# tiberiu44/TTS-Cube

Hardware: NVIDIA B200
Metric: audio samples/sec (higher is better)
Workload: dtype f32 in/out; tcgen05: fp16 hi*hi + 2 x fp8 (e4m3/e5m2) correction passes (GEMM1), split-fp16 x3 (GEMM2), f32 accumulate

## Files before the change

### include/cube_vocoder.h

```cpp
#ifndef CUBE_VOCODER_H_
#define CUBE_VOCODER_H_

#include <stdint.h>

#ifdef __cplusplus
extern "C" {
#endif

typedef struct cube_voc cube_voc_t;
typedef void* cube_stream_t;

enum cube_voc_arch {
  CUBE_VOC_HIFIGAN = 0,
  CUBE_VOC_PWN_STUDENT = 1,
  CUBE_VOC_WAVERNN = 2,
  CUBE_VOC_UPSAMPLENET = 3
};

enum cube_wavernn_head { CUBE_HEAD_MOL = 0, CUBE_HEAD_GM = 1, CUBE_HEAD_MULAW = 2, CUBE_HEAD_RAW = 3 };

enum cube_voc_math {
  CUBE_MATH_FP32_SIMT = 0,
  CUBE_MATH_TC_SPLIT16 = 1
};

#define CUBE_MAX_UPS 8
#define CUBE_MAX_RBK 8
#define CUBE_MAX_DIL 8
#define CUBE_MAX_FLOWS 8

typedef struct cube_voc_config {
  uint32_t struct_size;
  int32_t arch;
  int32_t math;
  int32_t num_mels;
  int32_t upsample_initial_channel;
  int32_t n_ups;
  int32_t upsample_rates[CUBE_MAX_UPS];
  int32_t upsample_kernel_sizes[CUBE_MAX_UPS];
  int32_t resblock_type;
  int32_t n_resblock_kernels;
  int32_t resblock_kernel_sizes[CUBE_MAX_RBK];
  int32_t n_dilations[CUBE_MAX_RBK];
  int32_t resblock_dilations[CUBE_MAX_RBK][CUBE_MAX_DIL];
  int32_t n_flows;
  int32_t flow_blocks[CUBE_MAX_FLOWS];
  int32_t res_channels, gate_channels, skip_channels;
  int32_t kernel_size, front_kernel;
  int32_t dilation_base, dilation_cycle;
  int32_t n_upsample;
  int32_t upsample_scales[4];
  int32_t wrnn_layers, wrnn_size;
  int32_t wrnn_upsample, wrnn_upsample_low;
  int32_t wrnn_use_lowres;
  int32_t wrnn_head;
} cube_voc_config;

int cube_voc_create(cube_voc_t** out, const cube_voc_config* cfg, int device);

int cube_voc_load_weight(cube_voc_t* h, const char* name, const float* data, const int64_t* shape, int ndim);

int cube_voc_finalize(cube_voc_t* h);

int64_t cube_voc_out_len(const cube_voc_t* h, int64_t n_frames);

int cube_voc_forward(cube_voc_t* h, const float* mel, const int32_t* n_frames, const float* noise,
                     float* wav, int16_t* wav_i16, int B, int64_t Fmax, cube_stream_t stream);

int cube_voc_hifigan_support(const cube_voc_config* cfg, int64_t s0, int64_t s1, int64_t* f0, int64_t* f1);

int cube_voc_forward_range(cube_voc_t* h, const float* mel, const int32_t* n_frames, const int64_t* out_begin,
                           const int64_t* out_end, float* wav, int16_t* wav_i16, int B, int64_t Fmax, cube_stream_t stream);

int cube_voc_forward_host(cube_voc_t* h, const float* mel, const int32_t* n_frames, const float* noise,
                          float* wav, int16_t* wav_i16, int B, int64_t Fmax);

int64_t cube_wavernn_out_len(const cube_voc_t* h, int64_t n_frames, int64_t n_low);
int cube_wavernn_forward(cube_voc_t* h, const float* mel, const float* x_low, const float* draws, float* x,
                         int B, int64_t F, int64_t Tl, cube_stream_t stream);
int cube_wavernn_max_batch(const cube_voc_t* h);

int cube_voc_get_cond(cube_voc_t* h, float* c_up, int B, int64_t Tmax, cube_stream_t stream);

int64_t cube_voc_last_launches(const cube_voc_t* h);
int64_t cube_voc_workspace_bytes(const cube_voc_t* h);
int cube_voc_set_profile(cube_voc_t* h, int on);
int cube_voc_get_profile(cube_voc_t* h, char* names , float* ms, int cap);

void cube_voc_destroy(cube_voc_t* h);
const char* cube_voc_last_error(void);
const char* cube_voc_build_info(void);

int cube_mulaw_encode(const float* x, int64_t* q, int64_t n, cube_stream_t stream);
int cube_mulaw_decode(const int64_t* q, float* x, int64_t n, cube_stream_t stream);
int cube_raw_encode(const float* x, int64_t* q, int64_t n, cube_stream_t stream);
int cube_raw_decode(const int64_t* q, float* x, int64_t n, cube_stream_t stream);
int cube_mol_sample(const float* y, const float* u_mix, const float* u_x, float* x, int64_t n,
                    int nr_mix, float log_scale_min, float temperature, cube_stream_t stream);
int cube_gaussian_sample(const float* y, const float* eps, float* x, int64_t n, cube_stream_t stream);
int cube_categorical_sample(const float* logits, const float* u, int64_t* idx, int64_t n, int C,
                            cube_stream_t stream);
int cube_wav_to_int16(const float* wav, int16_t* out, int64_t n, cube_stream_t stream);

typedef struct cube_mel cube_mel_t;

typedef struct cube_mel_config {
  uint32_t struct_size;
  int32_t n_fft;
  int32_t win_size;
  int32_t hop_size;
  int32_t n_mels;
  int32_t pad_left;
  int32_t pad_right;
  int32_t log10_out;
  int32_t layout;
  int32_t pad_mode;
  float mag_eps;
  float floor_val;
  float pad_value;
  float preemph;
} cube_mel_config;

int cube_mel_create(cube_mel_t** out, const cube_mel_config* cfg, const float* window, const float* mel_basis, int device);
int64_t cube_mel_out_frames(const cube_mel_t* h, int64_t n_samples);
int cube_mel_forward(cube_mel_t* h, const float* wav, const int32_t* n_samples, float* mel, int B, int64_t Tmax,
                     int64_t Fmax, cube_stream_t stream);
void cube_mel_destroy(cube_mel_t* h);

#ifdef __cplusplus
}
#endif
#endif
```

### tts_cube_b200/_lib.py

```python
from __future__ import annotations

import ctypes as C
import os

_HERE = os.path.dirname(os.path.abspath(__file__))
LIB_PATH = os.path.join(_HERE, "libcube_vocoder.so")

MAX_UPS, MAX_RBK, MAX_DIL, MAX_FLOWS = 8, 8, 8, 8
ARCH_HIFIGAN, ARCH_PWN_STUDENT, ARCH_WAVERNN, ARCH_UPSAMPLENET = 0, 1, 2, 3
HEADS = {"mol": 0, "gm": 1, "mulaw": 2, "raw": 3}
MATH_FP32_SIMT, MATH_TC_SPLIT16 = 0, 1


class VocConfig(C.Structure):
    _fields_ = [
        ("struct_size", C.c_uint32),
        ("arch", C.c_int32), ("math", C.c_int32), ("num_mels", C.c_int32),
        ("upsample_initial_channel", C.c_int32), ("n_ups", C.c_int32),
        ("upsample_rates", C.c_int32 * MAX_UPS), ("upsample_kernel_sizes", C.c_int32 * MAX_UPS),
        ("resblock_type", C.c_int32), ("n_resblock_kernels", C.c_int32),
        ("resblock_kernel_sizes", C.c_int32 * MAX_RBK), ("n_dilations", C.c_int32 * MAX_RBK),
        ("resblock_dilations", (C.c_int32 * MAX_DIL) * MAX_RBK),
        ("n_flows", C.c_int32), ("flow_blocks", C.c_int32 * MAX_FLOWS),
        ("res_channels", C.c_int32), ("gate_channels", C.c_int32), ("skip_channels", C.c_int32),
        ("kernel_size", C.c_int32), ("front_kernel", C.c_int32),
        ("dilation_base", C.c_int32), ("dilation_cycle", C.c_int32),
        ("n_upsample", C.c_int32), ("upsample_scales", C.c_int32 * 4),
        ("wrnn_layers", C.c_int32), ("wrnn_size", C.c_int32), ("wrnn_upsample", C.c_int32),
        ("wrnn_upsample_low", C.c_int32), ("wrnn_use_lowres", C.c_int32), ("wrnn_head", C.c_int32),
    ]

    def __init__(self, *a, **k):
        super().__init__(*a, **k)
        self.struct_size = C.sizeof(VocConfig)


class MelConfig(C.Structure):
    _fields_ = [("struct_size", C.c_uint32),
                ("n_fft", C.c_int32), ("win_size", C.c_int32), ("hop_size", C.c_int32), ("n_mels", C.c_int32),
                ("pad_left", C.c_int32), ("pad_right", C.c_int32), ("log10_out", C.c_int32), ("layout", C.c_int32),
                ("pad_mode", C.c_int32),
                ("mag_eps", C.c_float), ("floor_val", C.c_float), ("pad_value", C.c_float), ("preemph", C.c_float)]

    def __init__(self, *a, **k):
        super().__init__(*a, **k)
        self.struct_size = C.sizeof(MelConfig)


class CubeVocError(RuntimeError):
    pass


_lib = None

_P = C.c_void_p
SYMBOLS = {
    "cube_voc_create": (C.c_int, [C.POINTER(_P), C.POINTER(VocConfig), C.c_int]),
    "cube_voc_load_weight": (C.c_int, [_P, C.c_char_p, _P, C.POINTER(C.c_int64), C.c_int]),
    "cube_voc_finalize": (C.c_int, [_P]),
    "cube_voc_out_len": (C.c_int64, [_P, C.c_int64]),
    "cube_voc_forward": (C.c_int, [_P, _P, _P, _P, _P, _P, C.c_int, C.c_int64, _P]),
    "cube_voc_forward_host": (C.c_int, [_P, _P, _P, _P, _P, _P, C.c_int, C.c_int64]),
    "cube_voc_hifigan_support": (C.c_int, [C.POINTER(VocConfig), C.c_int64, C.c_int64, C.POINTER(C.c_int64),
                                           C.POINTER(C.c_int64)]),
    "cube_voc_forward_range": (C.c_int, [_P, _P, _P, C.POINTER(C.c_int64), C.POINTER(C.c_int64), _P, _P, C.c_int,
                                         C.c_int64, _P]),
    "cube_voc_get_cond": (C.c_int, [_P, _P, C.c_int, C.c_int64, _P]),
    "cube_wavernn_out_len": (C.c_int64, [_P, C.c_int64, C.c_int64]),
    "cube_wavernn_forward": (C.c_int, [_P, _P, _P, _P, _P, C.c_int, C.c_int64, C.c_int64, _P]),
    "cube_wavernn_max_batch": (C.c_int, [_P]),
    "cube_voc_last_launches": (C.c_int64, [_P]),
    "cube_voc_workspace_bytes": (C.c_int64, [_P]),
    "cube_voc_set_profile": (C.c_int, [_P, C.c_int]),
    "cube_voc_get_profile": (C.c_int, [_P, _P, _P, C.c_int]),
    "cube_voc_destroy": (None, [_P]),
    "cube_voc_last_error": (C.c_char_p, []),
    "cube_voc_build_info": (C.c_char_p, []),
    "cube_mulaw_encode": (C.c_int, [_P, _P, C.c_int64, _P]),
    "cube_mulaw_decode": (C.c_int, [_P, _P, C.c_int64, _P]),
    "cube_raw_encode": (C.c_int, [_P, _P, C.c_int64, _P]),
    "cube_raw_decode": (C.c_int, [_P, _P, C.c_int64, _P]),
    "cube_mol_sample": (C.c_int, [_P, _P, _P, _P, C.c_int64, C.c_int, C.c_float, C.c_float, _P]),
    "cube_gaussian_sample": (C.c_int, [_P, _P, _P, C.c_int64, _P]),
    "cube_categorical_sample": (C.c_int, [_P, _P, _P, C.c_int64, C.c_int, _P]),
    "cube_wav_to_int16": (C.c_int, [_P, _P, C.c_int64, _P]),
    "cube_mel_create": (C.c_int, [C.POINTER(_P), C.POINTER(MelConfig), _P, _P, C.c_int]),
    "cube_mel_out_frames": (C.c_int64, [_P, C.c_int64]),
    "cube_mel_forward": (C.c_int, [_P, _P, C.POINTER(C.c_int32), _P, C.c_int, C.c_int64, C.c_int64, _P]),
    "cube_mel_destroy": (None, [_P]),
}


def lib() -> C.CDLL:
    global _lib
    if _lib is None:
        if not os.path.exists(LIB_PATH):
            raise CubeVocError(
                f"{LIB_PATH} not found - build it with `python -c 'import __graft_entry__ as g; g.build()'` "
                "(nvcc, sm_100a).  tts_cube_b200 has no CPU or PyTorch fallback.")
        l = C.CDLL(LIB_PATH)
        for name, (res, args) in SYMBOLS.items():
            fn = getattr(l, name)
            fn.restype = res
            fn.argtypes = args
        _lib = l
    return _lib


def check(rc: int) -> None:
    if rc != 0:
        raise CubeVocError(lib().cube_voc_last_error().decode("utf-8", "replace"))


def build_info() -> str:
    return lib().cube_voc_build_info().decode()
```

### tts_cube_b200/csrc/engine.cu

```cuda
#include <cuda_runtime.h>
#include <math.h>
#include <stdarg.h>
#include <stdio.h>
#include <string.h>

#include <map>
#include <string>
#include <vector>

#include "../../include/cube_vocoder.h"
#include "conv_simt.cuh"
#include "heads.cuh"
#include "tc_conv.cuh"
#include "tc_block.cuh"
#include "tc_rbstep.cuh"
#include "wavernn.cuh"
#include "melspec.cuh"

#define CUBE_VERSION "0.1.0"
#ifndef CUBE_FUSED_DEFAULT
#define CUBE_FUSED_DEFAULT true
#endif

namespace cube {

static thread_local char g_err[1024] = "";

static int fail(const char* fmt, ...) {
  va_list ap;
  va_start(ap, fmt);
  vsnprintf(g_err, sizeof(g_err), fmt, ap);
  va_end(ap);
  return 1;
}

#define CU_TRY(expr)                                                                       \
  do {                                                                                     \
    cudaError_t _e = (expr);                                                               \
    if (_e != cudaSuccess)                                                                 \
      return fail("%s failed: %s (%s:%d)", #expr, cudaGetErrorString(_e), __FILE__, __LINE__); \
  } while (0)

struct HostTensor {
  std::vector<int64_t> shape;
  std::vector<float> data;
  int64_t numel() const { int64_t n = 1; for (auto s : shape) n *= s; return n; }
};

struct DevBuf {
  float* p = nullptr;
  size_t bytes = 0;
};

struct PackedConv {
  float* W = nullptr;
  float* bias = nullptr;
  int M = 0, Mpad = 0, Ktot = 0, nphase = 1;
};

struct ProfRec { std::string name; cudaEvent_t a, b; };

struct TcPacked {
  __half* Wimg = nullptr;
  uint8_t* Wimg8 = nullptr;
  float* inv_scale = nullptr;
  float* bias = nullptr;
  int N = 0, n_tiles = 0, nchunks_total = 0, nseg = 0;
  int bn = 256, nphase = 1;
  long long w_phase_stride = 0;
  tc::TcSeg seg[2];
};

}

using namespace cube;

struct cube_voc {
  cube_voc_config cfg;
  int device = 0;
  bool finalized = false;
  std::map<std::string, HostTensor> host_w;
  std::vector<void*> dev_allocs;
  std::map<std::string, DevBuf> ws;
  int* d_lens = nullptr; size_t lens_cap = 0;
  std::vector<int> h_lens;
  void* hs_in = nullptr; size_t hs_in_cap = 0;
  float* d_mel = nullptr; size_t d_mel_cap = 0;
  float* d_noise = nullptr; size_t d_noise_cap = 0;
  float* d_wav = nullptr; size_t d_wav_cap = 0;
  int16_t* d_wav16 = nullptr; size_t d_wav16_cap = 0;
  cudaStream_t own_stream = nullptr;
  int64_t launches = 0;
  struct GraphEntry { cudaGraphExec_t exec = nullptr; uint64_t gen = 0; int64_t launches = 0; int seen = 0; };
  std::map<std::vector<int64_t>, GraphEntry> graphs;
  uint64_t alloc_gen = 0;
  int* h_lens_pin = nullptr; size_t h_lens_pin_cap = 0;
  bool lens_from_pinned = false;
  int sm_count = 148;
  bool profile = false;
  std::vector<ProfRec> prof;
  PackedConv conv_pre, conv_post_w;
  std::vector<PackedConv> ups;
  std::vector<std::vector<PackedConv>> rb_c1, rb_c2;
  TcPacked tc_conv_pre;
  std::vector<TcPacked> tc_ups;
  std::vector<std::vector<TcPacked>> tc_c1, tc_c2;
  struct Flow {
    PackedConv front, final1, final3;
    std::vector<PackedConv> gate, resskip;
    std::vector<TcPacked> tc_gate, tc_resskip;
    TcPacked tc_final1;
    TcPacked tc_front;
    bool has_tc_front = false;
    float* w3 = nullptr;
  };
  std::vector<Flow> flows;
  struct Up2 { float w[192]; float bias; int s; };
  std::vector<Up2> up2;
  struct Wrnn {
    PackedConv lowres[3], gx;
    float *w_last = nullptr, *whh1 = nullptr, *bhh1 = nullptr, *wih2 = nullptr, *bih2 = nullptr, *whh2 = nullptr, *bhh2 = nullptr;
    float *wpre = nullptr, *bpre = nullptr, *wout = nullptr, *bout = nullptr;
    int S = 0, ic = 0;
  } wr;
  struct UpNet { PackedConv conv[3]; std::vector<PackedConv> up; std::vector<int> J; } upnet;
  int last_B = 0; int64_t last_T = 0;
  std::vector<int> h_rng;
};

namespace cube {

static int dev_upload(cube_voc* h, const std::vector<float>& v, float** out) {
  float* d = nullptr;
  CU_TRY(cudaMalloc(&d, std::max<size_t>(v.size(), 1) * sizeof(float)));
  CU_TRY(cudaMemcpy(d, v.data(), v.size() * sizeof(float), cudaMemcpyHostToDevice));
  h->dev_allocs.push_back(d);
  *out = d;
  return 0;
}

static int ws_get(cube_voc* h, const char* name, size_t n_floats, float** out) {
  DevBuf& b = h->ws[name];
  const size_t need = n_floats * sizeof(float);
  if (b.bytes < need) {
    if (b.p) CU_TRY(cudaFree(b.p));
    b.p = nullptr; b.bytes = 0;
    ++h->alloc_gen;
    CU_TRY(cudaMalloc(&b.p, need));
    b.bytes = need;
  }
  *out = b.p;
  return 0;
}

static int get_weight(cube_voc* h, const std::string& base, HostTensor* out) {
  auto it = h->host_w.find(base + ".weight");
  if (it != h->host_w.end()) { *out = it->second; return 0; }
  auto ig = h->host_w.find(base + ".weight_g"), iv = h->host_w.find(base + ".weight_v");
  if (ig == h->host_w.end() || iv == h->host_w.end()) return fail("missing weight '%s.weight[_g/_v]'", base.c_str());
  const HostTensor& g = ig->second; const HostTensor& v = iv->second;
  const int64_t n0 = v.shape[0], inner = v.numel() / n0;
  if (g.numel() != n0) return fail("weight_g of '%s' has %lld elements, expected %lld", base.c_str(), (long long)g.numel(), (long long)n0);
  out->shape = v.shape;
  out->data.resize(v.data.size());
  for (int64_t i = 0; i < n0; ++i) {
    double ss = 0;
    for (int64_t j = 0; j < inner; ++j) { double x = v.data[i * inner + j]; ss += x * x; }
    const float scale = (float)((double)g.data[i] / sqrt(ss));
    for (int64_t j = 0; j < inner; ++j) out->data[i * inner + j] = v.data[i * inner + j] * scale;
  }
  return 0;
}

static int get_bias(cube_voc* h, const std::string& base, int64_t n, const HostTensor** out) {
  auto it = h->host_w.find(base + ".bias");
  if (it == h->host_w.end()) return fail("missing '%s.bias'", base.c_str());
  if (it->second.numel() != n) return fail("'%s.bias' has %lld elements, expected %lld", base.c_str(), (long long)it->second.numel(), (long long)n);
  *out = &it->second;
  return 0;
}

static int expect_shape(const std::string& name, const HostTensor& t, std::initializer_list<int64_t> s) {
  std::vector<int64_t> e(s);
  if (t.shape != e) {
    std::string got, exp;
    for (auto x : t.shape) got += std::to_string(x) + ",";
    for (auto x : e) exp += std::to_string(x) + ",";
    return fail("weight '%s' has shape [%s], expected [%s]", name.c_str(), got.c_str(), exp.c_str());
  }
  return 0;
}

static inline int round_up(int x, int m) { return (x + m - 1) / m * m; }

static int pack_conv1d(cube_voc* h, const std::string& base, int M, int C, int K, PackedConv* pc) {
  HostTensor w; const HostTensor* b;
  if (get_weight(h, base, &w)) return 1;
  if (expect_shape(base, w, {M, C, K})) return 1;
  if (get_bias(h, base, M, &b)) return 1;
  pc->M = M; pc->Mpad = round_up(M, 128); pc->Ktot = C * K; pc->nphase = 1;
  std::vector<float> P((size_t)pc->Ktot * pc->Mpad, 0.f), B(pc->Mpad, 0.f);
  for (int m = 0; m < M; ++m) {
    B[m] = b->data[m];
    for (int c = 0; c < C; ++c)
      for (int k = 0; k < K; ++k) P[(size_t)(c * K + k) * pc->Mpad + m] = w.data[((size_t)m * C + c) * K + k];
  }
  if (dev_upload(h, P, &pc->W)) return 1;
  return dev_upload(h, B, &pc->bias);
}

static int pack_convT(cube_voc* h, const std::string& base, int C, int M, int K, int u, PackedConv* pc, int* J_out) {
  HostTensor w; const HostTensor* b;
  if (get_weight(h, base, &w)) return 1;
  if (expect_shape(base, w, {C, M, K})) return 1;
  if (get_bias(h, base, M, &b)) return 1;
  const int J = (K + u - 1) / u;
  pc->M = M; pc->Mpad = round_up(M, 128); pc->Ktot = C * J; pc->nphase = u;
  std::vector<float> P((size_t)u * pc->Ktot * pc->Mpad, 0.f), B(pc->Mpad, 0.f);
  for (int m = 0; m < M; ++m) B[m] = b->data[m];
  for (int r = 0; r < u; ++r)
    for (int c = 0; c < C; ++c)
      for (int jj = 0; jj < J; ++jj) {
        const int k = r + (J - 1 - jj) * u;
        if (k >= K) continue;
        for (int m = 0; m < M; ++m)
          P[((size_t)r * pc->Ktot + (size_t)c * J + jj) * pc->Mpad + m] = w.data[((size_t)c * M + m) * K + k];
      }
  *J_out = J;
  if (dev_upload(h, P, &pc->W)) return 1;
  return dev_upload(h, B, &pc->bias);
}

static int pack_small(cube_voc* h, const std::string& base, int M, int C, int K, PackedConv* pc) {
  HostTensor w; const HostTensor* b;
  if (get_weight(h, base, &w)) return 1;
  if (expect_shape(base, w, {M, C, K})) return 1;
  if (get_bias(h, base, M, &b)) return 1;
  pc->M = M; pc->Mpad = M; pc->Ktot = C * K;
  std::vector<float> P((size_t)C * K * M), B(M);
  for (int m = 0; m < M; ++m) {
    B[m] = b->data[m];
    for (int c = 0; c < C; ++c)
      for (int k = 0; k < K; ++k) P[(size_t)(c * K + k) * M + m] = w.data[((size_t)m * C + c) * K + k];
  }
  if (dev_upload(h, P, &pc->W)) return 1;
  return dev_upload(h, B, &pc->bias);
}

static int dev_upload_bytes(cube_voc* h, const void* src, size_t bytes, void** out) {
  void* d = nullptr;
  CU_TRY(cudaMalloc(&d, std::max<size_t>(bytes, 16)));
// ... 611 lines not shown
  if (ws_get(h, "hA", stage_max * B, &bufA) || ws_get(h, "hB", stage_max * B, &bufB) ||
      ws_get(h, "hC", stage_max * B, &bufC) || ws_get(h, "hD", stage_max * B, &bufD)) return 1;
  Launcher lx{h, st};
  const float LR = 0.1f;

  {
    lx.begin("conv_pre");
    ConvP p = make_conv(h->conv_pre);
    p.nseg = 1;
    p.seg[0] = make_seg(mel, (long long)c.num_mels * Fmax, c.num_mels, (int)Fmax, 7, 1, -3, PRE_NONE, 0.f, h->d_lens);
    p.Q = (int)L[0]; p.L_out = (int)L[0]; p.out_lens = h->d_lens;
    p.out = bufD; p.out_bstride = (long long)C0 * L[0];
    lx.conv(p, B);
    lx.end();
  }
  int ch = C0;
  float* stage_in = bufD;
  for (int i = 0; i < nU; ++i) {
    const int u = c.upsample_rates[i], K = c.upsample_kernel_sizes[i], pad = (K - u) / 2;
    const int J = (K + u - 1) / u;
    const int Lin = (int)L[i], Lo = (int)L[i + 1];
    const int cho = ch / 2;
    const int* lens_in = h->d_lens + (size_t)i * B;
    const int* lens_out = h->d_lens + (size_t)(i + 1) * B;
    float *xu = bufA, *xt = bufB, *xr = bufC, *xs = bufD;
    {
      lx.begin("ups");
      ConvP p = make_conv(h->ups[i]);
      p.nseg = 1;
      p.seg[0] = make_seg(stage_in, (long long)ch * Lin, ch, Lin, J, 1, -(J - 1), PRE_LRELU, LR, lens_in);
      p.nphase = u; p.ostride = u;
      for (int r = 0; r < u; ++r) p.ooff[r] = r - pad;
      p.Q = (Lo - 1 + pad) / u + 1;
      p.L_out = Lo; p.out_lens = lens_out;
      p.out = xu; p.out_bstride = (long long)cho * Lo;
      lx.conv(p, B);
      lx.end();
    }
    ch = cho;
    const long long bs = (long long)ch * Lo;
    for (int j = 0; j < nk; ++j) {
      const int idx = i * nk + j, k = c.resblock_kernel_sizes[j], nd = c.n_dilations[j];
      const int accm = (j == 0) ? ACC_SET : (j == nk - 1 ? ACC_ADD_DIV : ACC_ADD);
      const float* xcur = xu;
      if (c.resblock_type == 1) {
        for (int m = 0; m < nd; ++m) {
          const int d = c.resblock_dilations[j][m];
          lx.begin("rb_conv1");
          ConvP p1 = make_conv(h->rb_c1[idx][m]);
          p1.nseg = 1;
          p1.seg[0] = make_seg(xcur, bs, ch, Lo, k, d, -((k * d - d) / 2), PRE_LRELU, LR);
          p1.Q = Lo; p1.L_out = Lo; p1.out_lens = lens_out; p1.out = xt; p1.out_bstride = bs;
          lx.conv(p1, B);
          lx.end();
          lx.begin("rb_conv2");
          ConvP p2 = make_conv(h->rb_c2[idx][m]);
          p2.nseg = 1;
          p2.seg[0] = make_seg(xt, bs, ch, Lo, k, 1, -((k - 1) / 2), PRE_LRELU, LR);
          p2.Q = Lo; p2.L_out = Lo; p2.out_lens = lens_out;
          p2.epi = EPI_RESADD; p2.res = xcur; p2.res_bstride = bs;
          const bool last = (m == nd - 1);
          p2.out = last ? nullptr : xr; p2.out_bstride = bs;
          if (last) { p2.acc = xs; p2.acc_bstride = bs; p2.acc_mode = accm; p2.acc_div = (float)nk; }
          if (last && nk == 1) { p2.acc_mode = ACC_SET; }
          lx.conv(p2, B);
          lx.end();
          xcur = xr;
        }
      } else {
        float* pp[2] = {xt, xr};
        for (int m = 0; m < nd; ++m) {
          const int d = c.resblock_dilations[j][m];
          lx.begin("rb2_conv");
          ConvP p1 = make_conv(h->rb_c1[idx][m]);
          p1.nseg = 1;
          p1.seg[0] = make_seg(xcur, bs, ch, Lo, k, d, -((k * d - d) / 2), PRE_LRELU, LR);
          p1.Q = Lo; p1.L_out = Lo; p1.out_lens = lens_out;
          p1.epi = EPI_RESADD; p1.res = xcur; p1.res_bstride = bs;
          const bool last = (m == nd - 1);
          p1.out = last ? nullptr : pp[m & 1]; p1.out_bstride = bs;
          if (last) { p1.acc = xs; p1.acc_bstride = bs; p1.acc_mode = (nk == 1) ? ACC_SET : accm; p1.acc_div = (float)nk; }
          lx.conv(p1, B);
          lx.end();
          xcur = pp[m & 1];
        }
      }
    }
    stage_in = xs;
  }
  {
    lx.begin("conv_post");
    const int Lo = (int)L[nU];
    SmallP p;
    memset(&p, 0, sizeof(p));
    p.src = stage_in; p.bstride = (long long)ch * Lo; p.C = ch; p.L = Lo;
    p.taps = 7; p.dil = 1; p.off0 = -3; p.preact = PRE_LRELU; p.slope = 0.01f;
    p.W = h->conv_post_w.W; p.bias = h->conv_post_w.bias;
    p.out_lens = h->d_lens + (size_t)nU * B; p.L_out = Lo;
    p.out = wav; p.out_bstride = Lo; p.out_i16 = wav16; p.epi = SEPI_TANH;
    if (rq) { p.row0 = (int)rq->s0; p.nrows = (int)(rq->s1 - rq->s0); p.out_rng = rq->d_rng; }
    lx.small(p, B, 1);
    lx.end();
  }
  return lx.err;
}

static bool use_win(const cube_voc* h) {
  static int v = -2;
  if (v == -2) { const char* e = getenv("CUBE_TC_WIN"); v = e ? (e[0] == '1' ? 1 : 0) : -1; }
  if (v >= 0) return v == 1;
  return h->cfg.arch == CUBE_VOC_HIFIGAN;
}

static bool block_stats_on() {
  static int v = -1;
  if (v < 0) { const char* e = getenv("CUBE_BLOCK_STATS"); v = (e && e[0] == '1') ? 1 : 0; }
  return v == 1;
}
static unsigned long long* block_stats_buf() {
  static unsigned long long* buf = nullptr;
  if (!buf) { cudaMalloc(&buf, 32 * sizeof(unsigned long long)); cudaMemset(buf, 0, 32 * sizeof(unsigned long long)); }
  return buf;
}
static void block_stats_dump(cudaStream_t st) {
  if (!block_stats_on()) return;
  unsigned long long v[32];
  cudaStreamSynchronize(st);
  cudaMemcpy(v, block_stats_buf(), sizeof(v), cudaMemcpyDeviceToHost);
  cudaMemset(block_stats_buf(), 0, sizeof(v));
  static const char* names[27] = {"prod.wait_empty_g1", "prod.wait_empty_g2", "prod.total",
    "mma.wait_accfree_g1a", "mma.wait_accfree_g1b", "mma.wait_full_g1", "mma.wait_accfree_g2", "mma.wait_ofull_kh0", "mma.wait_ofull_kh1",
    "mma.wait_full_g2", "mma.total",
    "epiR.wait_accfull_nt0", "epiR.wait_accfull_nt1", "epiR.wait_ofree_nt0", "epiR.wait_ofree_nt1", "epiR.wait_accfull_rs", "epiR.gate_math",
    "epiR.resskip", "epiR.-",
    "epiS.wait_accfull_nt0", "epiS.wait_accfull_nt1", "epiS.wait_ofree_nt0", "epiS.wait_ofree_nt1", "epiS.wait_accfull_rs", "epiS.gate_math",
    "epiS.resskip", "epiS.-"};
  fprintf(stderr, "[cube block stats] CTA 0, cycles summed over the forward:\n");
  for (int i = 0; i < 27; ++i) fprintf(stderr, "  %-24s %14llu  (%.1f %% of mma.total)\n", names[i], v[i], 100.0 * (double)v[i] / (double)(v[10] ? v[10] : 1));
}

static bool use_fused() {
  static int v = -2;
  if (v == -2) { const char* e = getenv("CUBE_TC_FUSED"); v = e ? (e[0] == '1' ? 1 : 0) : -1; }
  return v < 0 ? CUBE_FUSED_DEFAULT : v == 1;
}

#ifndef CUBE_LEAN_DEFAULT
#define CUBE_LEAN_DEFAULT 1
#endif
static bool use_lean() {
  static int v = -1;
  if (v < 0) { const char* e = getenv("CUBE_TC_LEAN"); v = e ? (e[0] == '1' ? 1 : 0) : CUBE_LEAN_DEFAULT; }
  return v == 1;
}

static bool use_cg2() {
  static int v = -1;
  if (v < 0) { const char* e = getenv("CUBE_TC_CG2"); v = (e && e[0] == '1') ? 1 : 0; }
  return v == 1;
}

static bool use_rbstep() {
  static int v = -1;
  if (v < 0) { const char* e = getenv("CUBE_TC_RBFUSE"); v = (e && e[0] == '0') ? 0 : 1; }
  return v == 1;
}

#ifndef CUBE_RB_PK_DEFAULT
#define CUBE_RB_PK_DEFAULT 0
#endif
static bool use_rb_pk() {
  static int v = -1;
  if (v < 0) { const char* e = getenv("CUBE_RB_PK"); v = e ? (e[0] == '1' ? 1 : 0) : CUBE_RB_PK_DEFAULT; }
  return v == 1;
}

template <int C, int NSUB, bool PK>
static int launch_rbstep_v(cube_voc* h, tc::RbParams& rp, cudaStream_t st) {
  using Cfg = tc::RbCfg<C, NSUB>;
  static bool attr[64] = {false};
  if (!attr[h->device & 63]) {
    CU_TRY(cudaFuncSetAttribute(tc::tc_rbstep_kernel<C, NSUB, PK>, cudaFuncAttributeMaxDynamicSharedMemorySize, Cfg::SMEM));
    attr[h->device & 63] = true;
  }
  const int r_out = NSUB * tc::BM - (rp.k - 1);
  rp.t_tiles = ((rp.nrows > 0 ? rp.nrows : rp.L) + r_out - 1) / r_out;
  const long long tiles = (long long)rp.t_tiles * rp.B;
  const int grid = (int)std::min<long long>(tiles, h->sm_count);
  tc::tc_rbstep_kernel<C, NSUB, PK><<<grid, tc::RB_THREADS, Cfg::SMEM, st>>>(rp);
  return 0;
}
template <int C, int NSUB>
static int launch_rbstep(cube_voc* h, tc::RbParams& rp, cudaStream_t st) {
  return use_rb_pk() ? launch_rbstep_v<C, NSUB, true>(h, rp, st) : launch_rbstep_v<C, NSUB, false>(h, rp, st);
}

#ifndef CUBE_WIDE_DEFAULT
#define CUBE_WIDE_DEFAULT 1
#endif
static int wide_mode() {
  static int v = -1;
  if (v < 0) { const char* e = getenv("CUBE_TC_WIDE"); v = e ? (e[0] == '2' ? 2 : (e[0] == '1' ? 1 : 0)) : CUBE_WIDE_DEFAULT; }
  return v;
}
static bool use_wide() { return wide_mode() > 0; }

template <int TN, int MS = 0>
static void launch_tc_t(cube_voc* h, tc::TcParams& tp, cudaStream_t st) {
  const int nph = tp.nphase > 0 ? tp.nphase : 1;
  const int rows = tp.nrows > 0 ? tp.nrows : tp.T;
  if (MS == 0 && use_cg2()) {
    static bool attr2[64] = {false};
    if (!attr2[h->device & 63]) {
      cudaFuncSetAttribute(tc::tc_conv_kernel<TN, true>, cudaFuncAttributeMaxDynamicSharedMemorySize, tc::Cfg<TN, true>::SMEM);
      attr2[h->device & 63] = true;
    }
    constexpr int rows2 = 2 * tc::BM * tc::Cfg<TN, true>::MSUB;
    tp.t_tiles = (rows + rows2 - 1) / rows2;
    const long long tiles = (long long)tp.n_tiles * tp.t_tiles * tp.B * nph;
    cudaLaunchConfig_t cfg;
    memset(&cfg, 0, sizeof(cfg));
    cfg.gridDim = dim3(2 * (unsigned)std::min<long long>(tiles, h->sm_count / 2));
    cfg.blockDim = dim3(tc::NUM_THREADS);
    cfg.dynamicSmemBytes = tc::Cfg<TN, true>::SMEM;
    cfg.stream = st;
    cudaLaunchAttribute at[1];
    at[0].id = cudaLaunchAttributeClusterDimension;
    at[0].val.clusterDim.x = 2; at[0].val.clusterDim.y = 1; at[0].val.clusterDim.z = 1;
    cfg.attrs = at; cfg.numAttrs = 1;
    cudaLaunchKernelEx(&cfg, tc::tc_conv_kernel<TN, true>, tp);
    return;
  }
  constexpr int rows1 = tc::BM * tc::Cfg<TN, false, MS>::MSUB;
  tp.t_tiles = (rows + rows1 - 1) / rows1;
  const long long tiles = (long long)tp.n_tiles * tp.t_tiles * tp.B * nph;
  const int grid = (int)std::min<long long>(tiles, h->sm_count);
  if (use_win(h)) {
    tc::TcParams wp = tp;
    wp.nseg = 0;
    wp.lean = use_lean() ? 1 : 0;
    int base = 0;
    bool ok = true;
    for (int s_ = 0; s_ < tp.nseg && ok; ++s_) {
      const tc::TcSeg sg = tp.seg[s_];
      const int span = (sg.taps - 1) * sg.dil;
      if (span <= tc::BM) {
        if (wp.nseg >= tc::MAX_SEG) { ok = false; break; }
        tc::TcSeg n = sg;
        n.src = s_; n.wchunk0 = base; n.nbox = (rows1 + span + tc::BM - 1) / tc::BM;
        wp.seg[wp.nseg++] = n;
      } else {
        for (int j = 0; j < sg.taps; ++j) {
          if (wp.nseg >= tc::MAX_SEG) { ok = false; break; }
          tc::TcSeg n = sg;
          n.taps = 1; n.off0 = sg.off0 + j * sg.dil; n.src = s_; n.wchunk0 = base + j * sg.nchunks; n.nbox = rows1 / tc::BM;
          wp.seg[wp.nseg++] = n;
        }
      }
      base += sg.taps * sg.nchunks;
    }
    if (ok) {
      static bool attrw[64] = {false};
      if (!attrw[h->device & 63]) {
        cudaFuncSetAttribute(tc::tc_conv_kernel<TN, false, true, MS>, cudaFuncAttributeMaxDynamicSharedMemorySize, tc::WinCfg<TN, MS>::SMEM);
        attrw[h->device & 63] = true;
      }
      tc::tc_conv_kernel<TN, false, true, MS><<<grid, tc::NUM_THREADS, tc::WinCfg<TN, MS>::SMEM, st>>>(wp);
      return;
    }
  }
  static bool attr[64] = {false};
  if (!attr[h->device & 63]) {
    cudaFuncSetAttribute(tc::tc_conv_kernel<TN, false, false, MS>, cudaFuncAttributeMaxDynamicSharedMemorySize, tc::Cfg<TN, false, MS>::SMEM);
    attr[h->device & 63] = true;
  }
  tc::tc_conv_kernel<TN, false, false, MS><<<grid, tc::NUM_THREADS, tc::Cfg<TN, false, MS>::SMEM, st>>>(tp);
}

static bool wide_pays(const cube_voc* h, const tc::TcParams& tp) {
  const long long nph = tp.nphase > 0 ? tp.nphase : 1;
  const long long tiles128 = (long long)tp.n_tiles * ((tp.T + tc::BM - 1) / tc::BM) * tp.B * nph;
  return wide_mode() == 2 || tiles128 >= 2LL * h->sm_count;
}

static void launch_tc_bn(cube_voc* h, int bn, tc::TcParams& tp, cudaStream_t st) {
  if (bn == 256) launch_tc_t<256>(h, tp, st);
  else if (bn == 128 && use_wide() && use_win(h) && !use_cg2() && wide_pays(h, tp)) launch_tc_t<128, 2>(h, tp, st);
  else if (bn == 128) launch_tc_t<128>(h, tp, st);
  else if (bn == 64) launch_tc_t<64>(h, tp, st);
  else launch_tc_t<32>(h, tp, st);
}

static int forward_hifigan_tc(cube_voc* h, const float* mel, const int32_t* n_frames, float* wav, int16_t* wav16,
                              int B, int64_t Fmax, cudaStream_t st, const RangeReq* rq) {
  const cube_voc_config& c = h->cfg;
  const int nU = c.n_ups, nk = c.n_resblock_kernels;
  std::vector<int64_t> L(nU + 1);
  for (int i = 0; i <= nU; ++i) L[i] = hifigan_len(c, Fmax, i);
  if (L[nU] > 0x7fffffffLL / 2) return fail("utterance too long");
  HifiganPlan plan;
  if (rq) hifigan_plan(c, rq->s0, rq->s1, L.data(), true, &plan);
  auto crop = [&](auto& prm, RowRange r) {
    if (!rq) return;
    prm.row0 = (int)r.a; prm.nrows = (int)std::max<int64_t>(r.b - r.a, 1);
  };
  if (upload_lens(h, n_frames, B, Fmax, nU + 1, st)) return 1;
// ... 186 lines not shown
    const float* src = mel;
    int Lin = (int)Fmax, scale = 1;
    for (int n = 0; n < c.n_upsample; ++n) {
      lx.begin("upsample2d");
      Up2dP p;
      memset(&p, 0, sizeof(p));
      const int s = h->up2[n].s;
      p.src = src; p.out = (n == c.n_upsample - 1) ? cup : ((n & 1) ? cmid2 : cmid);
      p.src_lens = h->d_lens; p.lens_scale = scale;
      p.nf = CI; p.L_in = Lin; p.L_out = Lin * s; p.s = s; p.pad = s / 2;
      memcpy(p.w, h->up2[n].w, sizeof(p.w));
      p.bias = h->up2[n].bias; p.slope = 0.4f;
      if (s % 4 == 0 && p.pad % 4 == 0 && p.L_out % 4 == 0 && ((uintptr_t)p.out & 15) == 0) {
        dim3 grid((p.L_out / 4 + 255) / 256, CI, B);
        upsample2d_x4_kernel<<<grid, 256, 0, st>>>(p);
      } else {
        dim3 grid((p.L_out + 255) / 256, CI, B);
        upsample2d_kernel<<<grid, 256, 0, st>>>(p);
      }
      lx.check();
      lx.end();
      src = p.out; Lin = p.L_out; scale *= s;
    }
    if (c.n_upsample == 0) return fail("n_upsample must be >= 1");
  }
  h->last_B = B; h->last_T = T;
  const float* zin = noise;
  const float rs = sqrtf(0.5f);
  const bool use_tc = (c.math == CUBE_MATH_TC_SPLIT16);
  __half *h16 = nullptr, *h16b = nullptr, *o16 = nullptr, *c16 = nullptr, *s16 = nullptr, *zc16 = nullptr;
  uint8_t *h8 = nullptr, *h8b = nullptr, *c8 = nullptr;
  CUtensorMap tm_h, tm_hb, tm_o, tm_c, tm_s, tm_h32, tm_hb32, tm_z, tm_h8, tm_h8b, tm_c8;
  const bool fp8 = use_tc && use_fused() && use_fp8();
  if (use_tc) {
    float *t1, *t2, *t3, *t4;
    if (ws_get(h, "s16", (size_t)B * T * S, &t4)) return 1;
    s16 = (__half*)t4;
    if (make_tmap_hl16(&tm_s, s16, B, T, S)) return 1;
    if (use_fused()) {
      float* t5;
      if (ws_get(h, "h16b", (size_t)B * T * R, &t5)) return 1;
      h16b = (__half*)t5;
      if (make_tmap_hl16(&tm_hb, h16b, B, T, R) || make_tmap_hl16(&tm_hb32, h16b, B, T, R, 32)) return 1;
    }
    if (ws_get(h, "h16", (size_t)B * T * R, &t1) || ws_get(h, "o16", (size_t)B * T * G, &t2) ||
        ws_get(h, "c16", (size_t)B * T * CI, &t3)) return 1;
    h16 = (__half*)t1; o16 = (__half*)t2; c16 = (__half*)t3;
    if (make_tmap_hl16(&tm_h, h16, B, T, R) || make_tmap_hl16(&tm_o, o16, B, T, G) || make_tmap_hl16(&tm_c, c16, B, T, CI)) return 1;
    if (use_fused() && make_tmap_hl16(&tm_h32, h16, B, T, R, 32)) return 1;
    if (c.front_kernel % tc::BK == 0) {
      float* t6;
      if (ws_get(h, "zc16", (size_t)B * T * c.front_kernel, &t6)) return 1;
      zc16 = (__half*)t6;
      if (make_tmap_hl16(&tm_z, zc16, B, T, c.front_kernel)) return 1;
    }
    lx.begin("to_hl16");
    tc::to_hl16_kernel<<<dim3((T + 31) / 32, (CI + 31) / 32, B), 256, 0, st>>>(cup, c16, B, CI, T);
    lx.check();
    lx.end();
    if (fp8) {
      float *u1, *u2, *u3;
      if (ws_get(h, "h8", (size_t)B * T * R / 2, &u1) || ws_get(h, "h8b", (size_t)B * T * R / 2, &u2) ||
          ws_get(h, "c8", (size_t)B * T * CI / 2, &u3)) return 1;
      h8 = (uint8_t*)u1; h8b = (uint8_t*)u2; c8 = (uint8_t*)u3;
      if (make_tmap_q8(&tm_h8, h8, B, T, R) || make_tmap_q8(&tm_h8b, h8b, B, T, R) || make_tmap_q8(&tm_c8, c8, B, T, CI)) return 1;
      lx.begin("to_q8");
      tc::hl16_to_q8_kernel<<<h->sm_count * 8, 256, 0, st>>>(c16, c8, (long long)B * T * CI);
      lx.check();
      lx.end();
    }
  }
  auto launch_tc = [&](const TcPacked& pk, tc::TcParams& tp) {
    tp.Wimg = pk.Wimg; tp.inv_scale = pk.inv_scale; tp.bias = pk.bias;
    tp.nseg = pk.nseg; tp.nchunks_total = pk.nchunks_total;
    tp.B = B; tp.T = T; tp.n_tiles = pk.n_tiles;
    tp.lens = lens_T;
    tp.nphase = 1; tp.a_inv_scale = 1.f; tp.plane_scale = 1.f;
    launch_tc_t<256>(h, tp, st);
    lx.check();
  };
  for (int f = 0; f < c.n_flows; ++f) {
    cube_voc::Flow& fl = h->flows[f];
    const bool last_flow = (f == c.n_flows - 1);
    float* zout = last_flow ? wav : ((f & 1) ? zb : za);
    if (use_tc && fl.has_tc_front) {
      lx.begin("front_tc");
      tc::taps_to_hl16_kernel<<<h->sm_count * 8, 256, 0, st>>>(zin, zc16, B, T, c.front_kernel);
      lx.check();
      tc::TcParams tp;
      memset(&tp, 0, sizeof(tp));
      tp.tmA[0] = tm_z; tp.tmA[1] = tm_z;
      tp.Wimg = fl.tc_front.Wimg; tp.inv_scale = fl.tc_front.inv_scale; tp.bias = fl.tc_front.bias;
      tp.nseg = 1; tp.seg[0] = fl.tc_front.seg[0]; tp.nchunks_total = fl.tc_front.nchunks_total;
      tp.B = B; tp.T = T; tp.n_tiles = fl.tc_front.n_tiles;
      tp.lens = lens_T; tp.epi = tc::TC_EPI_CONV; tp.out16 = h16; tp.outC = R; tp.L_out = T;
      tp.nphase = 1; tp.ostride = 1; tp.out_slope = 0.f; tp.res_inv_slope = 1.f; tp.acc_div = 1.f;
      tp.a_inv_scale = 1.f; tp.plane_scale = 1.f;
      launch_tc_t<128>(h, tp, st);
      lx.check();
      lx.end();
      if (fp8) {
        lx.begin("to_q8");
        tc::hl16_to_q8_kernel<<<h->sm_count * 8, 256, 0, st>>>(h16, h8, (long long)B * T * R);
        lx.check();
        lx.end();
      }
    } else {
      lx.begin("front");
      ConvP p = make_conv(fl.front);
      p.nseg = 1;
      p.seg[0] = make_seg(zin, T, 1, T, c.front_kernel, 1, -(c.front_kernel - 1), PRE_NONE, 0.f, lens_T);
      p.Q = T; p.L_out = T; p.out_lens = lens_T; p.post = POST_RELU;
      p.out = use_tc ? y1 : hb; p.out_bstride = (long long)R * T;
      lx.conv(p, B);
      lx.end();
      if (use_tc) {
        lx.begin("to_hl16");
        tc::to_hl16_kernel<<<dim3((T + 31) / 32, (R + 31) / 32, B), 256, 0, st>>>(y1, h16, B, R, T);
        lx.check();
        lx.end();
      }
    }
    const int nb = c.flow_blocks[f];
    for (int i = 0; i < nb; ++i) {
      const int d = dilation_of(c, i);
      if (use_tc && use_fused() && K * (R / tc::BK) + (CI + tc::BK - 1) / tc::BK == fl.tc_gate[i].nchunks_total && G == 256 && T % 4 == 0) {
        lx.begin("block_fused");
        tc::BlockParams bp;
        memset(&bp, 0, sizeof(bp));
        bp.tmH = tm_h; bp.tmC = tm_c;
        bp.tmHin32 = tm_h32; bp.tmHout32 = tm_hb32;
        bp.h_in16 = h16; bp.h_out16 = h16b;
        bp.W1 = fl.tc_gate[i].Wimg; bp.inv1 = fl.tc_gate[i].inv_scale; bp.bias1 = fl.tc_gate[i].bias;
        bp.W2 = fl.tc_resskip[i].Wimg; bp.inv2 = fl.tc_resskip[i].inv_scale; bp.bias2 = fl.tc_resskip[i].bias;
        bp.taps = K; bp.dil = d; bp.off0 = -(K - 1) * d;
        bp.h_chunks = R / tc::BK; bp.c_chunks = (CI + tc::BK - 1) / tc::BK;
        bp.c_last_ksteps = ((CI - (bp.c_chunks - 1) * tc::BK) + 15) / 16;
        bp.B = B; bp.T = T; bp.t_tiles = (T + tc::BM - 1) / tc::BM;
        bp.lens = lens_T; bp.skip = sk; bp.skip_set = (i == 0); bp.scale = rs;
        bp.skip16 = (i == nb - 1) ? s16 : nullptr;
        const bool q8 = fp8 && fl.has_tc_front && fl.tc_gate[i].Wimg8;
        if (q8) { bp.tmH8 = tm_h8; bp.tmC8 = tm_c8; bp.W1q = fl.tc_gate[i].Wimg8; bp.h8_out = h8b; bp.h8_in = h8; bp.c8_in = c8; }
        static int pfn = -1;
        if (pfn < 0) { const char* e = getenv("CUBE_TC_PREFETCH"); pfn = (e && e[0] == '1') ? 1 : 0; }
        bp.prefetch_next = pfn; bp.c_in16 = c16; bp.c_ch = CI;
        bp.lean = use_lean() ? 1 : 0;
        static int pairv = -1;
        if (pairv < 0) { const char* e = getenv("CUBE_TC_PAIR"); pairv = (e && e[0] == '0') ? 0 : 1; }
        const bool stats = block_stats_on();
        if (stats) bp.stats = block_stats_buf();
        static int aonce = -1;
        if (aonce < 0) { const char* e = getenv("CUBE_TC_AONCE"); aonce = (e && e[0] == '1') ? 1 : 0; }
        const bool use_aonce = pairv == 1 && aonce == 1 && !stats;
        auto launch = [&](auto kernel, bool pair) -> int {
          const size_t smem = use_aonce ? tc::AONCE_SMEM : (pair ? tc::PAIR_SMEM : tc::BLK_SMEM);
          static std::map<std::pair<const void*, int>, bool> attr_done;
          const auto key = std::make_pair((const void*)kernel, h->device);
          if (!attr_done[key]) {
            CU_TRY(cudaFuncSetAttribute(kernel, cudaFuncAttributeMaxDynamicSharedMemorySize, (int)smem));
            attr_done[key] = true;
          }
          cudaLaunchConfig_t cfg;
          memset(&cfg, 0, sizeof(cfg));
          cudaLaunchAttribute at[1];
          if (pair) {
            bp.t_tiles = (T + 2 * tc::BM - 1) / (2 * tc::BM);
            const long long ptiles = (long long)bp.t_tiles * B;
            cfg.gridDim = dim3(2 * (unsigned)std::min<long long>(ptiles, h->sm_count / 2));
            at[0].id = cudaLaunchAttributeClusterDimension;
            at[0].val.clusterDim.x = 2; at[0].val.clusterDim.y = 1; at[0].val.clusterDim.z = 1;
            cfg.attrs = at; cfg.numAttrs = 1;
          } else {
            const long long tiles = (long long)bp.t_tiles * B;
            cfg.gridDim = dim3((unsigned)std::min<long long>(tiles, h->sm_count));
          }
          cfg.blockDim = dim3(tc::NUM_THREADS);
          cfg.dynamicSmemBytes = smem;
          cfg.stream = st;
          CU_TRY(cudaLaunchKernelEx(&cfg, kernel, bp));
          return 0;
        };
        int lrc;
        if (use_aonce) {
          lrc = q8 ? launch(tc::tc_block_kernel<true, true, false, true>, true) : launch(tc::tc_block_kernel<true, false, false, true>, true);
        } else if (pairv == 1) {
          if (stats) lrc = q8 ? launch(tc::tc_block_kernel<true, true, true>, true) : launch(tc::tc_block_kernel<true, false, true>, true);
          else lrc = q8 ? launch(tc::tc_block_kernel<true, true, false>, true) : launch(tc::tc_block_kernel<true, false, false>, true);
        } else {
          if (stats) lrc = q8 ? launch(tc::tc_block_kernel<false, true, true>, false) : launch(tc::tc_block_kernel<false, false, true>, false);
          else lrc = q8 ? launch(tc::tc_block_kernel<false, true, false>, false) : launch(tc::tc_block_kernel<false, false, false>, false);
        }
        if (lrc) return 1;
        lx.check();
        lx.end();
        std::swap(h16, h16b);
        std::swap(tm_h, tm_hb);
        std::swap(tm_h32, tm_hb32);
        if (fp8) { std::swap(h8, h8b); std::swap(tm_h8, tm_h8b); }
        continue;
      }
      if (use_tc) {
        {
          lx.begin("gate");
          tc::TcParams tp;
          memset(&tp, 0, sizeof(tp));
          tp.tmA[0] = tm_h; tp.tmA[1] = tm_c;
          tp.seg[0] = fl.tc_gate[i].seg[0]; tp.seg[1] = fl.tc_gate[i].seg[1];
          tp.seg[0].dil = d; tp.seg[0].off0 = -(K - 1) * d;
          tp.epi = tc::TC_EPI_GATE; tp.out16 = o16; tp.outC = G;
          launch_tc(fl.tc_gate[i], tp);
          lx.end();
        }
        {
          lx.begin("resskip");
          tc::TcParams tp;
          memset(&tp, 0, sizeof(tp));
          tp.tmA[0] = tm_o; tp.tmA[1] = tm_o;
          tp.seg[0] = fl.tc_resskip[i].seg[0];
          tp.epi = tc::TC_EPI_RESSKIP; tp.h16 = h16; tp.hC = R; tp.skip = sk; tp.skip_set = (i == 0); tp.scale = rs;
          tp.skip16 = (i == nb - 1) ? s16 : nullptr;
          launch_tc(fl.tc_resskip[i], tp);
          lx.end();
        }
        continue;
      }
      {
        lx.begin("gate");
        ConvP p = make_conv(fl.gate[i]);
        p.nseg = 2;
        p.seg[0] = make_seg(hb, (long long)R * T, R, T, K, d, -(K - 1) * d, PRE_NONE, 0.f);
        p.seg[1] = make_seg(cup, (long long)CI * T, CI, T, 1, 1, 0, PRE_NONE, 0.f);
        p.Q = T; p.L_out = T; p.out_lens = lens_T; p.epi = EPI_GATE;
        p.out = ob; p.out_bstride = (long long)G * T;
        lx.conv(p, B);
        lx.end();
      }
      {
        lx.begin("resskip");
        ConvP p = make_conv(fl.resskip[i]);
        p.nseg = 1;
        p.seg[0] = make_seg(ob, (long long)G * T, G, T, 1, 1, 0, PRE_NONE, 0.f);
        p.Q = T; p.L_out = T; p.out_lens = lens_T; p.epi = EPI_RESSKIP;
        p.Mh = R; p.scale = rs;
        p.res = hb; p.res_bstride = (long long)R * T; p.out = hb; p.out_bstride = (long long)R * T;
        p.skip = sk; p.skip_bstride = (long long)S * T; p.skip_set = (i == 0);
        lx.conv(p, B);
        lx.end();
      }
    }
    if (use_tc) {
      lx.begin("final_iaf_tc");
      tc::TcParams tp;
      memset(&tp, 0, sizeof(tp));
      tp.tmA[0] = tm_s; tp.tmA[1] = tm_s;
      tp.seg[0] = fl.tc_final1.seg[0];
      tp.epi = tc::TC_EPI_FINAL; tp.w3 = fl.w3; tp.z_in = zin; tp.z_out = zout;
      launch_tc(fl.tc_final1, tp);
      lx.end();
      zin = zout;
      continue;
    }
    {
      lx.begin("final1");
      ConvP p = make_conv(fl.final1);
      p.nseg = 1;
      p.seg[0] = make_seg(sk, (long long)S * T, S, T, 1, 1, 0, PRE_RELU, 0.f);
      p.Q = T; p.L_out = T; p.out_lens = lens_T;
      p.out = y1; p.out_bstride = (long long)S * T;
      lx.conv(p, B);
      lx.end();
    }
    {
      lx.begin("final3_iaf");
      SmallP p;
      memset(&p, 0, sizeof(p));
      p.src = y1; p.bstride = (long long)S * T; p.C = S; p.L = T;
      p.taps = 1; p.dil = 1; p.off0 = 0; p.preact = PRE_RELU;
      p.W = fl.final3.W; p.bias = fl.final3.bias;
      p.out_lens = lens_T; p.L_out = T; p.out = zout; p.out_bstride = T;
      p.z = zin; p.z_bstride = T; p.epi = SEPI_IAF;
      lx.small(p, B, 2);
      lx.end();
    }
    zin = zout;
  }
  if (wav16 && !lx.err) {
    lx.begin("to_int16");
    const long long n = (long long)B * T;
    wav_to_int16_kernel<<<(int)std::min<long long>((n + 255) / 256, 148 * 16), 256, 0, st>>>(wav, wav16, n);
    lx.check();
    lx.end();
  }
  block_stats_dump(st);
  return lx.err;
}

static int get_tensor(cube_voc* h, const std::string& name, std::initializer_list<int64_t> shape, const HostTensor** out) {
  auto it = h->host_w.find(name);
  if (it == h->host_w.end()) return fail("missing '%s'", name.c_str());
  if (expect_shape(name, it->second, shape)) return 1;
  *out = &it->second;
  return 0;
}

static int wrnn_head_size(int head) { return head == CUBE_HEAD_MOL ? 30 : (head == CUBE_HEAD_GM ? 2 : 256); }

static int finalize_wavernn(cube_voc* h) {
  const cube_voc_config& c = h->cfg;
  const int H = c.wrnn_size, L = c.wrnn_layers, nm = c.num_mels;
  const int ic = nm + 1 + (c.wrnn_use_lowres ? 21 : 0);
  const int S = wrnn_head_size(c.wrnn_head);
  h->wr.S = S; h->wr.ic = ic;
  if (c.wrnn_use_lowres) {
    int ci = 1;
    for (int i = 0; i < 3; ++i) {
      if (pack_conv1d(h, "_lowres_conv." + std::to_string(i) + ".conv", 20, ci, 7, &h->wr.lowres[i])) return 1;
      ci = 20;
    }
  }
  const HostTensor *wih, *whh, *bih, *bhh;
  if (get_tensor(h, "_rnns.0.weight_ih_l0", {3 * H, ic}, &wih) || get_tensor(h, "_rnns.0.weight_hh_l0", {3 * H, H}, &whh) ||
      get_tensor(h, "_rnns.0.bias_ih_l0", {3 * H}, &bih) || get_tensor(h, "_rnns.0.bias_hh_l0", {3 * H}, &bhh)) return 1;
  {
    PackedConv& pc = h->wr.gx;
    pc.M = 3 * H; pc.Mpad = round_up(3 * H, 128); pc.Ktot = ic - 1; pc.nphase = 1;
    std::vector<float> P((size_t)pc.Ktot * pc.Mpad, 0.f), Bv(pc.Mpad, 0.f), wl(3 * H);
    for (int m = 0; m < 3 * H; ++m) {
      Bv[m] = bih->data[m];
      for (int k = 0; k < ic - 1; ++k) P[(size_t)k * pc.Mpad + m] = wih->data[(size_t)m * ic + k];
      wl[m] = wih->data[(size_t)m * ic + ic - 1];
    }
    if (dev_upload(h, P, &pc.W) || dev_upload(h, Bv, &pc.bias) || dev_upload(h, wl, &h->wr.w_last)) return 1;
  }
  if (dev_upload(h, whh->data, &h->wr.whh1) || dev_upload(h, bhh->data, &h->wr.bhh1)) return 1;
  if (L == 2) {
    const HostTensor *a, *b2, *c2, *d2;
    if (get_tensor(h, "_rnns.1.weight_ih_l0", {3 * H, H}, &a) || get_tensor(h, "_rnns.1.weight_hh_l0", {3 * H, H}, &b2) ||
        get_tensor(h, "_rnns.1.bias_ih_l0", {3 * H}, &c2) || get_tensor(h, "_rnns.1.bias_hh_l0", {3 * H}, &d2)) return 1;
    if (dev_upload(h, a->data, &h->wr.wih2) || dev_upload(h, b2->data, &h->wr.whh2) || dev_upload(h, c2->data, &h->wr.bih2) ||
        dev_upload(h, d2->data, &h->wr.bhh2)) return 1;
// ... 331 lines not shown
      return fail("bad upsample stage %d (rate %d, kernel %d)", i, cfg->upsample_rates[i], cfg->upsample_kernel_sizes[i]);
  for (int j = 0; j < cfg->n_resblock_kernels; ++j)
    if (cfg->resblock_kernel_sizes[j] < 1 || cfg->n_dilations[j] < 1 || cfg->n_dilations[j] > CUBE_MAX_DIL)
      return fail("bad ResBlock %d", j);
  if (s0 < 0 || s0 >= s1) return fail("empty or negative sample range [%lld, %lld)", (long long)s0, (long long)s1);
  HifiganPlan P;
  hifigan_plan(*cfg, s0, s1, nullptr, false, &P);
  *f0 = P.mel.a; *f1 = P.mel.b;
  return 0;
}

int cube_voc_forward_range(cube_voc_t* h, const float* mel, const int32_t* n_frames, const int64_t* out_begin,
                           const int64_t* out_end, float* wav, int16_t* wav_i16, int B, int64_t Fmax, cube_stream_t stream) {
  if (!h) return fail("null handle");
  if (h->cfg.arch != CUBE_VOC_HIFIGAN) return fail("the sample-range forward is defined for HiFi-GAN handles only");
  if (!h->finalized) return fail("forward before finalize");
  if (!mel || !wav || !out_begin || !out_end) return fail("null mel/wav/out_begin/out_end");
  if (B < 1 || Fmax < 1) return fail("empty batch (B=%d, Fmax=%lld)", B, (long long)Fmax);
  int64_t s0 = INT64_MAX, s1 = 0;
  h->h_rng.resize((size_t)2 * B);
  for (int b = 0; b < B; ++b) {
    const int64_t f = n_frames ? n_frames[b] : Fmax;
    if (f < 0 || f > Fmax) return fail("n_frames[%d]=%lld outside [0, %lld]", b, (long long)f, (long long)Fmax);
    const int64_t T = f == 0 ? 0 : hifigan_len(h->cfg, f, h->cfg.n_ups);
    if (out_begin[b] < 0 || out_begin[b] >= out_end[b] || out_end[b] > T)
      return fail("sample range [%lld, %lld) of item %d is empty or outside [0, %lld)", (long long)out_begin[b],
                  (long long)out_end[b], b, (long long)T);
    s0 = std::min(s0, out_begin[b]); s1 = std::max(s1, out_end[b]);
    h->h_rng[2 * b] = (int)out_begin[b]; h->h_rng[2 * b + 1] = (int)out_end[b];
  }
  if (hifigan_len(h->cfg, Fmax, h->cfg.n_ups) > 0x7fffffffLL / 2) return fail("utterance too long");
  if (ensure_device(h)) return 1;
  h->launches = 0;
  for (auto& r : h->prof) { cudaEventDestroy(r.a); cudaEventDestroy(r.b); }
  h->prof.clear();
  cudaStream_t st = (cudaStream_t)stream;
  float* d_rng;
  if (ws_get(h, "rng", (size_t)2 * B, &d_rng)) return 1;
  CU_TRY(cudaMemcpyAsync(d_rng, h->h_rng.data(), (size_t)2 * B * sizeof(int), cudaMemcpyHostToDevice, st));
  const RangeReq rq{s0, s1, (const int*)d_rng};
  return forward_hifigan(h, mel, n_frames, wav, wav_i16, B, Fmax, st, &rq);
}

static bool graphs_enabled() {
  static int v = -1;
  if (v < 0) { const char* e = getenv("CUBE_GRAPH"); v = (e && e[0] == '0') ? 0 : 1; }
  return v == 1;
}

int cube_voc_forward_host(cube_voc_t* h, const float* mel, const int32_t* n_frames, const float* noise, float* wav,
                          int16_t* wav_i16, int B, int64_t Fmax) {
  if (!h) return fail("null handle");
  if (!h->finalized) return fail("forward before finalize");
  if (!mel || (!wav && !wav_i16)) return fail("null mel / no output buffer");
  if (B < 1 || Fmax < 1) return fail("empty batch");
  if (h->cfg.arch == CUBE_VOC_WAVERNN) return fail("use cube_wavernn_forward for a WaveRNN handle");
  if (h->cfg.arch == CUBE_VOC_UPSAMPLENET) return fail("the host-buffer call is defined for the waveform vocoders; use cube_voc_forward for UpsampleNet");
  if (h->cfg.arch == CUBE_VOC_PWN_STUDENT && !noise) return fail("the IAF student needs `noise` (z ~ N(0,1), [B,1,T])");
  if (ensure_device(h)) return 1;
  const int64_t T = cube_voc_out_len(h, Fmax);
  const size_t mel_b = (size_t)B * h->cfg.num_mels * Fmax * sizeof(float);
  const size_t wav_n = (size_t)B * T;
  if (grow(&h->d_mel, &h->d_mel_cap, mel_b, &h->alloc_gen) || grow(&h->d_wav, &h->d_wav_cap, wav_n * sizeof(float), &h->alloc_gen)) return 1;
  if (wav_i16 && grow(&h->d_wav16, &h->d_wav16_cap, wav_n * sizeof(int16_t), &h->alloc_gen)) return 1;
  if (noise && grow(&h->d_noise, &h->d_noise_cap, wav_n * sizeof(float), &h->alloc_gen)) return 1;
  cudaStream_t st = h->own_stream;
  CU_TRY(cudaMemcpyAsync(h->d_mel, mel, mel_b, cudaMemcpyHostToDevice, st));
  if (noise) CU_TRY(cudaMemcpyAsync(h->d_noise, noise, wav_n * sizeof(float), cudaMemcpyHostToDevice, st));

  bool done = false;
  if (graphs_enabled() && !h->profile && !block_stats_on()) {
    const std::vector<int64_t> key = {B, Fmax, noise ? 1 : 0, wav_i16 ? 1 : 0};
    cube_voc::GraphEntry& ge = h->graphs[key];
    if (ge.exec && ge.gen != h->alloc_gen) { cudaGraphExecDestroy(ge.exec); ge.exec = nullptr; }
    if (ge.exec || ge.seen >= 1) {
      if (stage_lens_pinned(h, n_frames, B, Fmax)) return 1;
      if (ge.exec && ge.gen != h->alloc_gen) { cudaGraphExecDestroy(ge.exec); ge.exec = nullptr; }
    }
    if (!ge.exec && ge.seen >= 1) {
      const uint64_t gen0 = h->alloc_gen;
      cudaGraph_t graph = nullptr;
      h->lens_from_pinned = true;
      cudaError_t e = cudaStreamBeginCapture(st, cudaStreamCaptureModeThreadLocal);
      int rc = 1;
      if (e == cudaSuccess) {
        rc = cube_voc_forward(h, h->d_mel, n_frames, noise ? h->d_noise : nullptr, h->d_wav, wav_i16 ? h->d_wav16 : nullptr, B, Fmax, st);
        e = cudaStreamEndCapture(st, &graph);
      }
      h->lens_from_pinned = false;
      if (e == cudaSuccess && rc == 0 && graph && gen0 == h->alloc_gen) {
        cudaGraphExec_t ex = nullptr;
        if (cudaGraphInstantiate(&ex, graph, 0) == cudaSuccess) { ge.exec = ex; ge.gen = h->alloc_gen; ge.launches = h->launches; }
      }
      if (graph) cudaGraphDestroy(graph);
      if (!ge.exec) {
        cudaGetLastError();
        if (rc) return rc;
      }
    }
    if (ge.exec) {
      CU_TRY(cudaGraphLaunch(ge.exec, st));
      h->launches = ge.launches;
      done = true;
    }
    ++ge.seen;
  }
  if (!done && cube_voc_forward(h, h->d_mel, n_frames, noise ? h->d_noise : nullptr, h->d_wav, wav_i16 ? h->d_wav16 : nullptr, B, Fmax, st)) return 1;
  if (wav) CU_TRY(cudaMemcpyAsync(wav, h->d_wav, wav_n * sizeof(float), cudaMemcpyDeviceToHost, st));
  if (wav_i16) CU_TRY(cudaMemcpyAsync(wav_i16, h->d_wav16, wav_n * sizeof(int16_t), cudaMemcpyDeviceToHost, st));
  CU_TRY(cudaStreamSynchronize(st));
  return 0;
}

int64_t cube_wavernn_out_len(const cube_voc_t* h, int64_t n_frames, int64_t n_low) {
  if (!h || h->cfg.arch != CUBE_VOC_WAVERNN || n_frames < 0) { fail("bad argument"); return -1; }
  int64_t T = n_frames * h->cfg.wrnn_upsample;
  if (h->cfg.wrnn_use_lowres) T = std::min<int64_t>(T, n_low * h->cfg.wrnn_upsample_low);
  return T;
}

int cube_wavernn_max_batch(const cube_voc_t* h) {
  if (!h || h->cfg.arch != CUBE_VOC_WAVERNN || !h->finalized) { fail("bad handle"); return -1; }
  int b = 1;
  while (b < 1024 && wrnn_geom(h, b + 1).smem <= 227 * 1024) ++b;
  return b;
}

int cube_wavernn_forward(cube_voc_t* h, const float* mel, const float* x_low, const float* draws, float* x, int B, int64_t F,
                         int64_t Tl, cube_stream_t stream) {
  if (!h) return fail("null handle");
  if (h->cfg.arch != CUBE_VOC_WAVERNN) return fail("not a WaveRNN handle");
  if (!h->finalized) return fail("forward before finalize");
  if (!mel || !draws || !x) return fail("null argument");
  if (B < 1 || F < 1) return fail("empty batch");
  if (ensure_device(h)) return 1;
  h->launches = 0;
  for (auto& r : h->prof) { cudaEventDestroy(r.a); cudaEventDestroy(r.b); }
  h->prof.clear();
  return forward_wavernn(h, mel, x_low, draws, x, B, F, Tl, (cudaStream_t)stream);
}

int cube_voc_get_cond(cube_voc_t* h, float* c_up, int B, int64_t Tmax, cube_stream_t stream) {
  if (!h || !c_up) return fail("null argument");
  if (h->cfg.arch != CUBE_VOC_PWN_STUDENT) return fail("get_cond is only defined for the IAF student");
  if (B != h->last_B || Tmax != h->last_T) return fail("geometry differs from the last forward");
  auto it = h->ws.find("c_up");
  if (it == h->ws.end()) return fail("no forward has run");
  CU_TRY(cudaMemcpyAsync(c_up, it->second.p, (size_t)B * h->cfg.num_mels * Tmax * sizeof(float), cudaMemcpyDeviceToDevice, (cudaStream_t)stream));
  return 0;
}

int64_t cube_voc_last_launches(const cube_voc_t* h) { return h ? h->launches : -1; }

int64_t cube_voc_workspace_bytes(const cube_voc_t* h) {
  if (!h) return -1;
  int64_t n = 0;
  for (auto& kv : h->ws) n += (int64_t)kv.second.bytes;
  return n;
}

int cube_voc_set_profile(cube_voc_t* h, int on) {
  if (!h) return fail("null handle");
  h->profile = on != 0;
  return 0;
}

int cube_voc_get_profile(cube_voc_t* h, char* names, float* ms, int cap) {
  if (!h || !names || !ms) { fail("null argument"); return -1; }
  std::map<std::string, float> agg;
  std::vector<std::string> order;
  for (auto& r : h->prof) {
    if (cudaEventSynchronize(r.b) != cudaSuccess) { fail("profile event sync failed"); return -1; }
    float t = 0.f;
    cudaEventElapsedTime(&t, r.a, r.b);
    if (!agg.count(r.name)) order.push_back(r.name);
    agg[r.name] += t;
  }
  int n = 0;
  for (auto& k : order) {
    if (n >= cap) break;
    snprintf(names + (size_t)n * 64, 64, "%s", k.c_str());
    ms[n] = agg[k];
    ++n;
  }
  return n;
}

void cube_voc_destroy(cube_voc_t* h) {
  if (!h) return;
  cudaSetDevice(h->device);
  for (void* p : h->dev_allocs) cudaFree(p);
  for (auto& kv : h->ws) if (kv.second.p) cudaFree(kv.second.p);
  if (h->d_lens) cudaFree(h->d_lens);
  if (h->d_mel) cudaFree(h->d_mel);
  if (h->d_noise) cudaFree(h->d_noise);
  if (h->d_wav) cudaFree(h->d_wav);
  if (h->d_wav16) cudaFree(h->d_wav16);
  for (auto& r : h->prof) { cudaEventDestroy(r.a); cudaEventDestroy(r.b); }
  for (auto& kv : h->graphs) if (kv.second.exec) cudaGraphExecDestroy(kv.second.exec);
  if (h->h_lens_pin) cudaFreeHost(h->h_lens_pin);
  if (h->own_stream) cudaStreamDestroy(h->own_stream);
  delete h;
}

#define HEAD_PROLOGUE(n)                        \
  if ((n) < 0) return fail("negative length");  \
  if ((n) == 0) return 0;                       \
  if (tables_ready()) return 1;

int cube_mulaw_encode(const float* x, int64_t* q, int64_t n, cube_stream_t s) {
  HEAD_PROLOGUE(n);
  if (!x || !q) return fail("null argument");
  mulaw_encode_kernel<<<head_grid(n), 256, 0, (cudaStream_t)s>>>(x, (long long*)q, n);
  CU_TRY(cudaGetLastError());
  return 0;
}
int cube_mulaw_decode(const int64_t* q, float* x, int64_t n, cube_stream_t s) {
  HEAD_PROLOGUE(n);
  if (!x || !q) return fail("null argument");
  mulaw_decode_kernel<<<head_grid(n), 256, 0, (cudaStream_t)s>>>((const long long*)q, x, n);
  CU_TRY(cudaGetLastError());
  return 0;
}
int cube_raw_encode(const float* x, int64_t* q, int64_t n, cube_stream_t s) {
  HEAD_PROLOGUE(n);
  if (!x || !q) return fail("null argument");
  raw_encode_kernel<<<head_grid(n), 256, 0, (cudaStream_t)s>>>(x, (long long*)q, n);
  CU_TRY(cudaGetLastError());
  return 0;
}
int cube_raw_decode(const int64_t* q, float* x, int64_t n, cube_stream_t s) {
  HEAD_PROLOGUE(n);
  if (!x || !q) return fail("null argument");
  raw_decode_kernel<<<head_grid(n), 256, 0, (cudaStream_t)s>>>((const long long*)q, x, n);
  CU_TRY(cudaGetLastError());
  return 0;
}
int cube_mol_sample(const float* y, const float* u_mix, const float* u_x, float* x, int64_t n, int nr_mix,
                    float log_scale_min, float temperature, cube_stream_t s) {
  HEAD_PROLOGUE(n);
  if (!y || !u_mix || !u_x || !x) return fail("null argument");
  if (nr_mix < 1) return fail("nr_mix < 1");
  mol_sample_kernel<<<head_grid(n), 256, 0, (cudaStream_t)s>>>(y, u_mix, u_x, x, n, nr_mix, log_scale_min, temperature);
  CU_TRY(cudaGetLastError());
  return 0;
}
int cube_gaussian_sample(const float* y, const float* eps, float* x, int64_t n, cube_stream_t s) {
  HEAD_PROLOGUE(n);
  if (!y || !eps || !x) return fail("null argument");
  gaussian_sample_kernel<<<head_grid(n), 256, 0, (cudaStream_t)s>>>(y, eps, x, n);
  CU_TRY(cudaGetLastError());
  return 0;
}
int cube_categorical_sample(const float* logits, const float* u, int64_t* idx, int64_t n, int C, cube_stream_t s) {
  HEAD_PROLOGUE(n);
  if (!logits || !u || !idx) return fail("null argument");
  if (C < 1) return fail("C < 1");
  categorical_sample_kernel<<<head_grid(n * 32), 256, 0, (cudaStream_t)s>>>(logits, u, (long long*)idx, n, C);
  CU_TRY(cudaGetLastError());
  return 0;
}
int cube_wav_to_int16(const float* wav, int16_t* out, int64_t n, cube_stream_t s) {
  if (n < 0) return fail("negative length");
  if (n == 0) return 0;
  if (!wav || !out) return fail("null argument");
  wav_to_int16_kernel<<<head_grid(n), 256, 0, (cudaStream_t)s>>>(wav, out, n);
  CU_TRY(cudaGetLastError());
  return 0;
}

struct cube_mel {
  cube_mel_config cfg;
  int device = 0, n_bins = 0, KB = 0;
  float *cosT = nullptr, *sinT = nullptr, *basis = nullptr;
  int *k_lo = nullptr, *k_hi = nullptr, *d_len = nullptr;
  int len_cap = 0;
  size_t smem = 0;
};

int cube_mel_create(cube_mel_t** out, const cube_mel_config* cfg, const float* window, const float* mel_basis, int device) {
  using namespace cube;
  if (!out || !cfg || !mel_basis) return fail("null argument");
  if (cfg->struct_size != sizeof(cube_mel_config))
    return fail("cube_mel_config.struct_size = %u but this library's struct is %zu bytes: the binding does not match include/cube_vocoder.h",
                cfg->struct_size, sizeof(cube_mel_config));
  const cube_mel_config& c = *cfg;
  if (c.n_fft < 16 || c.n_fft > 4096 || c.n_fft % 4) return fail("n_fft must be a multiple of 4 in [16, 4096] (got %d)", c.n_fft);
  if (c.hop_size < 4 || c.hop_size % 4) return fail("hop_size must be a positive multiple of 4 (got %d)", c.hop_size);
  if (c.win_size < 1 || c.win_size > c.n_fft) return fail("win_size must be in [1, n_fft] (got %d)", c.win_size);
  if (c.n_mels < 1 || c.n_mels > 512) return fail("n_mels out of range (%d)", c.n_mels);
  if (c.pad_left < 0 || c.pad_right < 0) return fail("negative padding");
  if (c.layout != 0 && c.layout != 1) return fail("layout must be 0 ([B,M,F]) or 1 ([B,F,M])");
  if (c.pad_mode != 0 && c.pad_mode != 1) return fail("pad_mode must be 0 (reflect) or 1 (constant zeros)");
  int ndev = 0;
  if (cudaGetDeviceCount(&ndev) != cudaSuccess || ndev == 0) return fail("no CUDA device: libcube_vocoder has no CPU fallback");
  if (device < 0 || device >= ndev) return fail("device %d out of range (%d devices)", device, ndev);
  CU_TRY(cudaSetDevice(device));
  cube_mel* h = new cube_mel();
  h->cfg = c; h->device = device;
  h->n_bins = c.n_fft / 2 + 1;
  h->KB = (h->n_bins + mel::BT - 1) / mel::BT * mel::BT;
  h->smem = mel::smem_bytes(c.n_fft, c.hop_size, h->KB);
  if (h->smem > 220 * 1024) { delete h; return fail("n_fft/hop too large for one CTA's shared memory (%zu bytes)", h->smem); }
  const double PI = 3.14159265358979323846;
  std::vector<double> w(c.n_fft, 0.0);
  const int wl = (c.n_fft - c.win_size) / 2;
// ... 88 lines not shown
```

### tts_cube_b200/csrc/tc_block.cuh

```cuda
#pragma once
#include "tc_conv.cuh"

namespace cube {
namespace tc {

template <bool PAIR, bool AONCE = false> struct BlkCfg {
  static_assert(PAIR || !AONCE, "AONCE is a mode of the CTA-pair tiling");
  static constexpr int NST = AONCE ? 3 : (PAIR ? 4 : 3);
  static constexpr int B_BYTES = (PAIR ? 128 : 256) * BK * 2;
  static constexpr int STG = 2 * A_TILE_BYTES + (AONCE ? 4 : 2) * B_BYTES;
  static constexpr int O_BYTES = 2 * 4 * A_TILE_BYTES;
  static constexpr int SMEM = NST * STG + O_BYTES + 1024 + 512 + 768 * 8;
  static constexpr int TILE_ROWS = PAIR ? 2 * BM : BM;
};
constexpr int BLK_O_BYTES = BlkCfg<false>::O_BYTES;
constexpr int BLK_SMEM = BlkCfg<false>::SMEM;
constexpr int PAIR_SMEM = BlkCfg<true>::SMEM;
constexpr int AONCE_SMEM = BlkCfg<true, true>::SMEM;
static_assert(BK == 32, "tc_block_kernel is written for 32-channel K chunks (SWIZZLE_64B)");

struct BlockParams {
  CUtensorMap tmH, tmC;
  CUtensorMap tmHin32, tmHout32;
  const __half* W1;
  const __half* W2;
  const float* inv1; const float* bias1;
  const float* inv2; const float* bias2;
  int taps, dil, off0;
  int h_chunks, c_chunks, c_last_ksteps;
  int B, T, t_tiles;
  const int* lens;
  const __half* h_in16;
  __half* h_out16;
  float* skip; int skip_set; __half* skip16; float scale;
  CUtensorMap tmH8, tmC8;
  const uint8_t* W1q;
  uint8_t* h8_out;
  int prefetch_next;
  const __half* c_in16;
  const uint8_t* h8_in;
  const uint8_t* c8_in;
  int c_ch;
  unsigned long long* stats;
  int lean;
};

#define BLK_WAIT(bar, par, slot)                                   \
  do {                                                             \
    if (STATS) {                                                   \
      const long long _t0 = clock64();                             \
      mbar_wait(bar, par);                                         \
      st_acc[slot] += clock64() - _t0;                             \
    } else {                                                       \
      mbar_wait(bar, par);                                         \
    }                                                              \
  } while (0)

__device__ __forceinline__ void umma_f8_2(uint32_t tmem_d, uint64_t da, uint64_t db, uint32_t idesc, uint32_t accumulate) {
  asm volatile(
      "{\n\t"
      ".reg .pred p;\n\t"
      "setp.ne.b32 p, %4, 0;\n\t"
      "tcgen05.mma.cta_group::2.kind::f8f6f4 [%0], %1, %2, %3, p;\n\t"
      "}" ::"r"(tmem_d),
      "l"(da), "l"(db), "r"(idesc), "r"(accumulate)
      : "memory");
}
__device__ __forceinline__ void pair_arrive(uint64_t* bar, uint32_t crank) {
  if (crank == 0) mbar_arrive(bar); else mbar_arrive_remote(bar, 0);
}

template <bool PAIR>
__device__ __forceinline__ void blk_mma_f16(uint32_t d, uint64_t da, uint64_t db, uint32_t idesc, uint32_t acc) {
  if constexpr (PAIR) umma_f16_2(d, da, db, idesc, acc); else umma_f16(d, da, db, idesc, acc);
}
template <bool PAIR>
__device__ __forceinline__ void blk_mma_f8(uint32_t d, uint64_t da, uint64_t db, uint32_t idesc, uint32_t acc) {
  if constexpr (PAIR) umma_f8_2(d, da, db, idesc, acc); else umma_f8(d, da, db, idesc, acc);
}
template <bool PAIR>
__device__ __forceinline__ void blk_commit(uint64_t* bar) {
  if constexpr (PAIR) umma_commit_2(bar); else umma_commit(bar);
}

template <bool PAIR, bool Q8, bool STATS = false, bool AONCE = false>
__global__ void __launch_bounds__(NUM_THREADS, 1) tc_block_kernel(const __grid_constant__ BlockParams p) {
  long long st_acc[STATS ? 8 : 1] = {0};
  const long long st_begin = STATS ? clock64() : 0;
  (void)st_acc; (void)st_begin;
  constexpr int BN = 256;
  constexpr int B_BYTES = BlkCfg<PAIR, AONCE>::B_BYTES;
  constexpr int NST = BlkCfg<PAIR, AONCE>::NST;
  constexpr int STG = BlkCfg<PAIR, AONCE>::STG;
  constexpr int NPASS = AONCE ? 1 : 2;
  constexpr int NTP = AONCE ? 2 : 1;
  constexpr int TILE_ROWS = BlkCfg<PAIR>::TILE_ROWS;
  constexpr int NARR = PAIR ? 2 * NUM_EPI_WARPS : NUM_EPI_WARPS;
  const uint32_t crank = PAIR ? cluster_ctarank() : 0u;
  const int tile0 = PAIR ? (int)(blockIdx.x >> 1) : (int)blockIdx.x;
  const int tile_step = PAIR ? (int)(gridDim.x >> 1) : (int)gridDim.x;
  extern __shared__ uint8_t smem_raw[];
  uint8_t* smem = reinterpret_cast<uint8_t*>((reinterpret_cast<uintptr_t>(smem_raw) + 1023) & ~(uintptr_t)1023);
  uint8_t* o_smem = smem + NST * STG;
  uint64_t* bars = reinterpret_cast<uint64_t*>(o_smem + BlkCfg<PAIR, AONCE>::O_BYTES);
  uint64_t* full = bars;
  uint64_t* empty = bars + NST;
  uint64_t* pfull = bars + 2 * NST;
  uint64_t* acc_full = bars + 3 * NST;
  uint64_t* acc_free = acc_full + 2;
  uint64_t* o_full = acc_free + 2;
  uint64_t* o_free = o_full + 1;
  uint32_t* tmem_slot = reinterpret_cast<uint32_t*>(o_free + 1);
  uint64_t* hbar = o_free + 2;
  float2* sb1 = reinterpret_cast<float2*>(reinterpret_cast<uint8_t*>(bars) + 512);
  float2* sb2 = sb1 + 512;

  const int warp = threadIdx.x >> 5, lane = threadIdx.x & 31;
  const int total_tiles = p.t_tiles * p.B;
  const int nch1 = p.taps * p.h_chunks + p.c_chunks;

  if (warp == 0 && lane == 0) {
    prefetch_tmap(&p.tmH);
    prefetch_tmap(&p.tmC);
    for (int s = 0; s < NST; ++s) { mbar_init(&full[s], 1); mbar_init(&empty[s], 1); mbar_init(&pfull[s], 1); }
    for (int r = 0; r < 2; ++r) { mbar_init(&acc_full[r], 1); mbar_init(&acc_free[r], NARR); }
    mbar_init(o_full, NARR);
    mbar_init(o_free, 1);
    for (int w = 0; w < NUM_EPI_WARPS; ++w) mbar_init(&hbar[w], 1);
    prefetch_tmap(&p.tmHin32);
    prefetch_tmap(&p.tmHout32);
    if (Q8) { prefetch_tmap(&p.tmH8); prefetch_tmap(&p.tmC8); }
    fence_barrier_init();
  }
  if (warp == 1) { if constexpr (PAIR) tmem_alloc2(tmem_slot, 512); else tmem_alloc(tmem_slot, 512); }
  {
    constexpr float LOG2E = 1.4426950408889634f;
    for (int i = threadIdx.x; i < 512; i += NUM_THREADS) {
      const float k = (i & 255) < 128 ? 2.f * LOG2E : -LOG2E;
      sb1[i] = make_float2(__ldg(p.inv1 + i) * k, __ldg(p.bias1 + i) * k);
    }
    for (int i = threadIdx.x; i < 256; i += NUM_THREADS) sb2[i] = make_float2(__ldg(p.inv2 + i), __ldg(p.bias2 + i));
  }
  tc_fence_before();
  __syncthreads();
  if constexpr (PAIR) cluster_sync_all();
  tc_fence_after();
  const uint32_t tmem_base = *tmem_slot;

  if (warp == 0) {
    if (lane == 0) {
      uint32_t it = 0;
      for (int tile = tile0; tile < total_tiles; tile += tile_step) {
        const int tt = tile % p.t_tiles, b = tile / p.t_tiles;
        const int t0 = tt * TILE_ROWS + (int)crank * BM;
        for (int pass = 0; pass < NPASS; ++pass) {
          int chunk = 0;
          for (int tap = 0; tap <= p.taps; ++tap) {
            const bool cond = tap == p.taps;
            const int row = cond ? t0 : t0 + p.off0 + tap * p.dil;
            const int ncc = cond ? p.c_chunks : p.h_chunks;
            for (int cc = 0; cc < ncc; ++cc, ++chunk, ++it) {
              const int st = it % NST;
              BLK_WAIT(&empty[st], ((it / NST) & 1) ^ 1, 0);
              uint8_t* sb = smem + st * STG;
              const uint32_t fbar = smem_u32(&full[st]);
              mbar_expect_tx(&full[st], STG);
              const CUtensorMap* tm = cond ? &p.tmC : &p.tmH;
              tma_load_3d_bar(sb, tm, fbar, cc * BK, row, b);
              if constexpr (Q8) {
                const CUtensorMap* tm8 = cond ? &p.tmC8 : &p.tmH8;
                tma_load_3d_bar(sb + A_TILE_BYTES, tm8, fbar, cc * BK, row, b);
                tma_load_3d_bar(sb + A_TILE_BYTES + A_TILE_BYTES / 2, tm8, fbar, cc * BK, row, p.B + b);
              } else {
                tma_load_3d_bar(sb + A_TILE_BYTES, tm, fbar, cc * BK, row, p.B + b);
              }
#pragma unroll
              for (int k = 0; k < NTP; ++k) {
                const int nt = AONCE ? k : pass;
                uint8_t* wb = sb + 2 * A_TILE_BYTES + k * 2 * B_BYTES;
                if constexpr (Q8) {
                  const uint8_t* wq = p.W1q + ((size_t)nt * nch1 + chunk) * 32768;
                  bulk_load_bar(wb, wq + crank * B_BYTES, B_BYTES, fbar);
                  bulk_load_bar(wb + B_BYTES, wq + 16384 + crank * (B_BYTES / 2), B_BYTES / 2, fbar);
                  bulk_load_bar(wb + B_BYTES + B_BYTES / 2, wq + 24576 + crank * (B_BYTES / 2), B_BYTES / 2, fbar);
                } else {
                  const __half* wc = p.W1 + ((size_t)nt * nch1 + chunk) * 2 * (BN * BK) + (size_t)crank * (BN / 2) * BK ;
                  bulk_load_bar(wb, wc, B_BYTES, fbar);
                  bulk_load_bar(wb + B_BYTES, wc + BN * BK, B_BYTES, fbar);
                }
              }
            }
          }
        }
        for (int ch = 0; ch < 8; ++ch, ++it) {
          const int st = it % NST;
          BLK_WAIT(&empty[st], ((it / NST) & 1) ^ 1, 1);
          uint8_t* sb = smem + st * STG;
          const uint32_t fbar = smem_u32(&full[st]);
          mbar_expect_tx(&full[st], 2 * B_BYTES);
          const __half* wc = p.W2 + (size_t)ch * 2 * (BN * BK) + (size_t)crank * (BN / 2) * BK ;
          bulk_load_bar(sb + 2 * A_TILE_BYTES, wc, B_BYTES, fbar);
          bulk_load_bar(sb + 2 * A_TILE_BYTES + B_BYTES, wc + BN * BK, B_BYTES, fbar);
        }
      }
      if (STATS && p.stats && blockIdx.x == 0) {
        atomicAdd(p.stats + 0, (unsigned long long)st_acc[0]);
        atomicAdd(p.stats + 1, (unsigned long long)st_acc[1]);
        atomicAdd(p.stats + 2, (unsigned long long)(clock64() - st_begin));
      }
    }
  } else if (warp == 1) {
    if (crank == 0 && p.lean) {
      constexpr uint32_t idesc = make_idesc(BN, TILE_ROWS);
      constexpr uint32_t idesc8_0 = make_idesc_f8(BN, TILE_ROWS, 0), idesc8_1 = make_idesc_f8(BN, TILE_ROWS, 1);
      (void)idesc8_0; (void)idesc8_1;
      const uint64_t D16 = make_desc(smem_u32(smem)), D32 = make_desc32(smem_u32(smem));
      (void)D32;
      constexpr uint32_t O_OFF = NST * STG;
      constexpr uint32_t A8 = A_TILE_BYTES, AH = A_TILE_BYTES / 2, BH = B_BYTES / 2;
      (void)AH; (void)BH;
      const bool leader = elect_one();
      const uint32_t tmem_u = __shfl_sync(0xffffffffu, tmem_base, 0);
      uint32_t st = 0, ph = 0, titer = 0;
      uint32_t free_ph[2] = {0, 0};
      uint32_t ofull_ph = 0;
      for (int tile = tile0; tile < total_tiles; tile += tile_step, ++titer) {
        const int r0 = titer & 1, r1 = r0 ^ 1;
        for (int pass = 0; pass < NPASS; ++pass) {
#pragma unroll
          for (int k = 0; k < NTP; ++k) {
            const int rg = (AONCE ? k : pass) == 0 ? r0 : r1;
            BLK_WAIT(&acc_free[rg], (free_ph[rg] & 1) ^ 1, AONCE ? k : pass);
            ++free_ph[rg];
          }
          tc_fence_after();
          uint32_t accumulate = 0;
          for (int ch = 0; ch < nch1; ++ch) {
            BLK_WAIT(&full[st], ph, 2);
            if constexpr (PAIR) BLK_WAIT(&pfull[st], ph, 2);
            tc_fence_after();
            const uint32_t so = st * STG;
            const int ksteps = ch != nch1 - 1 ? BK / 16 : p.c_last_ksteps;
            if (leader) {
#pragma unroll
              for (int k = 0; k < NTP; ++k) {
                const int rg = (AONCE ? k : pass) == 0 ? r0 : r1;
                const uint32_t d_tmem = tmem_u + rg * BN;
                const uint32_t bo = so + 2 * A_TILE_BYTES + k * 2 * B_BYTES;
                if constexpr (Q8) {
                  blk_mma_f16<PAIR>(d_tmem, desc_add(D16, so), desc_add(D16, bo), idesc, accumulate);
                  if (ksteps > 1) blk_mma_f16<PAIR>(d_tmem, desc_add(D16, so + 32), desc_add(D16, bo + 32), idesc, 1);
                  blk_mma_f8<PAIR>(d_tmem, desc_add(D32, so + A8), desc_add(D32, bo + B_BYTES), idesc8_0, 1);
                  blk_mma_f8<PAIR>(d_tmem, desc_add(D32, so + A8 + AH), desc_add(D32, bo + B_BYTES + BH), idesc8_1, 1);
                } else {
#pragma unroll
                  for (int ks = 0; ks < BK / 16; ++ks) {
                    if (ks < ksteps) {
                      const uint32_t ko = ks * 32;
                      blk_mma_f16<PAIR>(d_tmem, desc_add(D16, so + ko), desc_add(D16, bo + ko), idesc, ks ? 1u : accumulate);
                      blk_mma_f16<PAIR>(d_tmem, desc_add(D16, so + ko), desc_add(D16, bo + B_BYTES + ko), idesc, 1);
                      blk_mma_f16<PAIR>(d_tmem, desc_add(D16, so + A8 + ko), desc_add(D16, bo + ko), idesc, 1);
                    }
                  }
                }
              }
              blk_commit<PAIR>(&empty[st]);
            }
            accumulate = 1;
            if (++st == NST) { st = 0; ph ^= 1; }
          }
          if (leader) {
#pragma unroll
            for (int k = 0; k < NTP; ++k) blk_commit<PAIR>(&acc_full[(AONCE ? k : pass) == 0 ? r0 : r1]);
          }
        }
        {
          BLK_WAIT(&acc_free[r0], (free_ph[r0] & 1) ^ 1, 3);
          ++free_ph[r0];
          const uint32_t d_tmem = tmem_u + r0 * BN;
          uint32_t accumulate = 0;
          for (int kh = 0; kh < 2; ++kh) {
            BLK_WAIT(o_full, ofull_ph & 1, 4 + kh);
            ++ofull_ph;
            tc_fence_after();
#pragma unroll 1
            for (int c4 = 0; c4 < 4; ++c4) {
              BLK_WAIT(&full[st], ph, 6);
              if constexpr (PAIR) BLK_WAIT(&pfull[st], ph, 6);
              tc_fence_after();
              const uint32_t ao = O_OFF + c4 * 2 * A_TILE_BYTES, bo = st * STG + 2 * A_TILE_BYTES;
              if (leader) {
#pragma unroll
                for (int ks = 0; ks < BK / 16; ++ks) {
                  const uint32_t ko = ks * 32;
                  blk_mma_f16<PAIR>(d_tmem, desc_add(D16, ao + ko), desc_add(D16, bo + ko), idesc, ks ? 1u : accumulate);
                  blk_mma_f16<PAIR>(d_tmem, desc_add(D16, ao + ko), desc_add(D16, bo + B_BYTES + ko), idesc, 1);
                  blk_mma_f16<PAIR>(d_tmem, desc_add(D16, ao + A8 + ko), desc_add(D16, bo + ko), idesc, 1);
                }
                blk_commit<PAIR>(&empty[st]);
              }
              accumulate = 1;
              if (++st == NST) { st = 0; ph ^= 1; }
            }
            if (leader) blk_commit<PAIR>(o_free);
          }
          if (leader) blk_commit<PAIR>(&acc_full[r0]);
        }
      }
      if (STATS && p.stats && blockIdx.x == 0 && leader) {
        for (int i = 0; i < 7; ++i) atomicAdd(p.stats + 3 + i, (unsigned long long)st_acc[i]);
        atomicAdd(p.stats + 10, (unsigned long long)(clock64() - st_begin));
      }
    } else if (lane == 0 && crank != 0) {
      uint32_t it = 0;
      for (int tile = tile0; tile < total_tiles; tile += tile_step)
        for (int n = NPASS * nch1 + 8; n > 0; --n, ++it) {
          const int st = it % NST;
          mbar_wait(&full[st], (it / NST) & 1);
          mbar_arrive_remote(&pfull[st], 0);
        }
    } else if (lane == 0) {
      constexpr uint32_t idesc = make_idesc(BN, TILE_ROWS);
      uint32_t it = 0, titer = 0;
      uint32_t free_ph[2] = {0, 0};
      uint32_t ofull_ph = 0;
      for (int tile = tile0; tile < total_tiles; tile += tile_step, ++titer) {
        const int r0 = titer & 1, r1 = r0 ^ 1;
        for (int pass = 0; pass < NPASS; ++pass) {
#pragma unroll
          for (int k = 0; k < NTP; ++k) {
            const int rg = (AONCE ? k : pass) == 0 ? r0 : r1;
            BLK_WAIT(&acc_free[rg], (free_ph[rg] & 1) ^ 1, AONCE ? k : pass);
            ++free_ph[rg];
          }
          tc_fence_after();
          uint32_t accumulate = 0;
          for (int tap = 0; tap <= p.taps; ++tap) {
            const bool cond = tap == p.taps;
            const int ncc = cond ? p.c_chunks : p.h_chunks;
            for (int cc = 0; cc < ncc; ++cc, ++it) {
              const int st = it % NST;
              BLK_WAIT(&full[st], (it / NST) & 1, 2);
              if constexpr (PAIR) BLK_WAIT(&pfull[st], (it / NST) & 1, 2);
              tc_fence_after();
              const uint32_t a_hi = smem_u32(smem + st * STG), a_lo = a_hi + A_TILE_BYTES;
              const int ksteps = (cond && cc == ncc - 1) ? p.c_last_ksteps : (BK / 16);
#pragma unroll
              for (int k = 0; k < NTP; ++k) {
                const int rg = (AONCE ? k : pass) == 0 ? r0 : r1;
                const uint32_t d_tmem = tmem_base + rg * BN;
                const uint32_t b_hi = a_hi + 2 * A_TILE_BYTES + k * 2 * B_BYTES, b_lo = b_hi + B_BYTES;
                uint32_t acc_k = accumulate;
                if constexpr (Q8) {
                  for (int ks = 0; ks < ksteps; ++ks) {
                    blk_mma_f16<PAIR>(d_tmem, make_desc(a_hi + ks * 32), make_desc(b_hi + ks * 32), idesc, acc_k);
                    acc_k = 1;
                  }
                  const uint32_t a8_hi = a_hi + A_TILE_BYTES, a8_lo = a8_hi + A_TILE_BYTES / 2;
                  const uint32_t b8_lo = b_hi + B_BYTES, b8_hi = b8_lo + B_BYTES / 2;
                  blk_mma_f8<PAIR>(d_tmem, make_desc32(a8_hi), make_desc32(b8_lo), make_idesc_f8(BN, TILE_ROWS, 0), 1);
                  blk_mma_f8<PAIR>(d_tmem, make_desc32(a8_lo), make_desc32(b8_hi), make_idesc_f8(BN, TILE_ROWS, 1), 1);
                } else {
                  for (int ks = 0; ks < ksteps; ++ks) {
                    const uint32_t ko = ks * 32;
                    blk_mma_f16<PAIR>(d_tmem, make_desc(a_hi + ko), make_desc(b_hi + ko), idesc, acc_k);
                    blk_mma_f16<PAIR>(d_tmem, make_desc(a_hi + ko), make_desc(b_lo + ko), idesc, 1);
                    blk_mma_f16<PAIR>(d_tmem, make_desc(a_lo + ko), make_desc(b_hi + ko), idesc, 1);
                    acc_k = 1;
                  }
                }
              }
              accumulate = 1;
              blk_commit<PAIR>(&empty[st]);
            }
          }
#pragma unroll
          for (int k = 0; k < NTP; ++k) blk_commit<PAIR>(&acc_full[(AONCE ? k : pass) == 0 ? r0 : r1]);
        }
        {
          BLK_WAIT(&acc_free[r0], (free_ph[r0] & 1) ^ 1, 3);
          ++free_ph[r0];
          const uint32_t d_tmem = tmem_base + r0 * BN;
          uint32_t accumulate = 0;
          for (int kh = 0; kh < 2; ++kh) {
            BLK_WAIT(o_full, ofull_ph & 1, 4 + kh);
            ++ofull_ph;
            tc_fence_after();
            for (int c4 = 0; c4 < 4; ++c4, ++it) {
              const int st = it % NST;
              BLK_WAIT(&full[st], (it / NST) & 1, 6);
              if constexpr (PAIR) BLK_WAIT(&pfull[st], (it / NST) & 1, 6);
              tc_fence_after();
              const uint32_t a_hi = smem_u32(o_smem + c4 * 2 * A_TILE_BYTES), a_lo = a_hi + A_TILE_BYTES;
              const uint32_t b_hi = smem_u32(smem + st * STG) + 2 * A_TILE_BYTES, b_lo = b_hi + B_BYTES;
              for (int ks = 0; ks < BK / 16; ++ks) {
                const uint32_t ko = ks * 32;
                blk_mma_f16<PAIR>(d_tmem, make_desc(a_hi + ko), make_desc(b_hi + ko), idesc, accumulate);
                blk_mma_f16<PAIR>(d_tmem, make_desc(a_hi + ko), make_desc(b_lo + ko), idesc, 1);
                blk_mma_f16<PAIR>(d_tmem, make_desc(a_lo + ko), make_desc(b_hi + ko), idesc, 1);
                accumulate = 1;
              }
              blk_commit<PAIR>(&empty[st]);
            }
            blk_commit<PAIR>(o_free);
          }
          blk_commit<PAIR>(&acc_full[r0]);
        }
      }
      if (STATS && p.stats && blockIdx.x == 0) {
        for (int i = 0; i < 7; ++i) atomicAdd(p.stats + 3 + i, (unsigned long long)st_acc[i]);
        atomicAdd(p.stats + 10, (unsigned long long)(clock64() - st_begin));
      }
    }
  } else {
    const int q = warp & 3;
    const int grp = (warp - 2) >> 2;
    const int row = q * 32 + lane;
    uint32_t titer = 0;
    uint32_t full_ph[2] = {0, 0};
    uint32_t ofree_ph = 0;
    for (int tile = tile0; tile < total_tiles; tile += tile_step, ++titer) {
      const int tt = tile % p.t_tiles, b = tile / p.t_tiles;
      const int t = tt * TILE_ROWS + (int)crank * BM + row;
      const int r0 = titer & 1, r1 = r0 ^ 1;
      const int len = p.lens ? min(p.lens[b], p.T) : p.T;
      const bool in_range = t < p.T, valid = t < len;
      if (p.prefetch_next && tile + tile_step < total_tiles) {
        const int ntile = tile + tile_step;
        const int ntt = ntile % p.t_tiles, nb = ntile / p.t_tiles;
        const int nt0 = ntt * TILE_ROWS + (int)crank * BM;
        const int e = (int)threadIdx.x - 64;
        const int rr = e & 127, part = e >> 7;
        const size_t hplane = (size_t)p.B * p.T * 128;
        for (int tap = 0; tap < p.taps; ++tap) {
          const int row = nt0 + p.off0 + tap * p.dil + rr;
          if (row >= 0 && row < p.T) {
            const size_t ro = (size_t)nb * p.T + row;
            if constexpr (Q8) {
              if (part < 2) prefetch_l2(p.h_in16 + ro * 128 + part * 64);
              else prefetch_l2(p.h8_in + (size_t)(part - 2) * hplane + ro * 128);
            } else {
              prefetch_l2(p.h_in16 + (size_t)(part >> 1) * hplane + ro * 128 + (part & 1) * 64);
            }
          }
        }
        const int crow = nt0 + rr;
        if (crow < p.T && p.c_in16) {
          const size_t ro = (size_t)nb * p.T + crow;
          const size_t cplane = (size_t)p.B * p.T * p.c_ch;
          if constexpr (Q8) {
            if (part < 2) prefetch_l2(p.c_in16 + ro * p.c_ch + part * 64);
            else if (p.c8_in) prefetch_l2(p.c8_in + (size_t)(part - 2) * cplane + ro * p.c_ch);
          } else {
            prefetch_l2(p.c_in16 + (size_t)(part >> 1) * cplane + ro * p.c_ch + (part & 1) * 64);
          }
        }
      }
      if (in_range && p.skip16 && !p.skip_set && (lane & 7) == 0) {
        const float* s0 = p.skip + ((size_t)b * 128 + grp * 32) * p.T + t;
#pragma unroll 8
        for (int j = 0; j < 32; ++j) prefetch_l2(s0 + (size_t)j * p.T);
      }
      for (int nt = 0; nt < 2; ++nt) {
        const int rg = nt == 0 ? r0 : r1;
        BLK_WAIT(&acc_full[rg], full_ph[rg] & 1, nt);
        ++full_ph[rg];
        const long long g_t0 = STATS ? clock64() : 0;
        tc_fence_after();
        const uint32_t taddr = tmem_base + rg * BN + ((uint32_t)(q * 32) << 16);
        const float2* sb = sb1 + nt * 256;
        uint8_t* otile = o_smem + grp * 2 * A_TILE_BYTES;
        uint32_t hi2[2][8], lo2[2][8];
#pragma unroll
        for (int ci = 0; ci < 2; ++ci) {
          const int cc = ci * 16;
          uint32_t f[16], g[16];
          tmem_ld16(taddr + grp * 32 + cc, f);
          tmem_ld16(taddr + 128 + grp * 32 + cc, g);
          tmem_ld_wait();
#pragma unroll
          for (int j = 0; j < 16; j += 2) {
            float o[2];
#pragma unroll
            for (int u = 0; u < 2; ++u) {
              const float2 sf = sb[grp * 32 + cc + j + u], sg = sb[128 + grp * 32 + cc + j + u];
              const float a = fminf(fmaxf(fmaf(__uint_as_float(f[j + u]), sf.x, sf.y), -40.f), 40.f);
              const float e = fminf(fmaf(__uint_as_float(g[j + u]), sg.x, sg.y), 60.f);
              const float E1 = ex2_fast(a), E2 = ex2_fast(e);
              o[u] = valid ? (E1 - 1.f) * rcp_fast((E1 + 1.f) * (1.f + E2)) : 0.f;
            }
            split16x2(o[0], o[1], hi2[ci][j >> 1], lo2[ci][j >> 1]);
          }
        }
        tc_fence_before();
        __syncwarp();
        if (lane == 0) pair_arrive(&acc_free[rg], crank);
        if (STATS) st_acc[5] += clock64() - g_t0;
        BLK_WAIT(o_free, (ofree_ph & 1) ^ 1, 2 + nt);
        ++ofree_ph;
        if (nt == 0) {
          asm volatile("cp.async.bulk.wait_group.read 0;" ::: "memory");
          __syncwarp();
        }
#pragma unroll
        for (int ci = 0; ci < 2; ++ci) {
#pragma unroll
          for (int v = 0; v < 2; ++v) {
            const int c16 = ci * 2 + v;
            const uint32_t off = row * 64 + ((c16 ^ ((row >> 1) & 3)) << 4);
            *reinterpret_cast<uint4*>(otile + off) = make_uint4(hi2[ci][4 * v], hi2[ci][4 * v + 1], hi2[ci][4 * v + 2], hi2[ci][4 * v + 3]);
            *reinterpret_cast<uint4*>(otile + A_TILE_BYTES + off) = make_uint4(lo2[ci][4 * v], lo2[ci][4 * v + 1], lo2[ci][4 * v + 2], lo2[ci][4 * v + 3]);
          }
        }
        fence_proxy_async();
        __syncwarp();
        if (lane == 0) pair_arrive(o_full, crank);
      }
      {
        const uint32_t taddr_rs = tmem_base + r0 * BN + ((uint32_t)(q * 32) << 16) + grp * 32;
        const size_t plane = (size_t)p.B * p.T * 128;
        float* sp0 = p.skip + ((size_t)b * 128 + grp * 32) * p.T + t;
        const bool last_block = p.skip16 != nullptr;
        const int ew = warp - 2;
        uint8_t* piece_hi = o_smem + grp * 2 * A_TILE_BYTES + q * 2048;
        uint8_t* piece_lo = piece_hi + A_TILE_BYTES;
        const int tw = tt * TILE_ROWS + (int)crank * BM + q * 32;
        float old[32];
        if (last_block) {
#pragma unroll
          for (int j = 0; j < 32; ++j) old[j] = (in_range && !p.skip_set) ? __ldcs(sp0 + (size_t)j * p.T) : 0.f;
        }
        BLK_WAIT(&acc_full[r0], full_ph[r0] & 1, 4);
        ++full_ph[r0];
        const long long r_t0 = STATS ? clock64() : 0;
        tc_fence_after();
        if (lane == 0) {
          mbar_expect_tx(&hbar[ew], 2 * 2048);
          tma_load_3d(piece_hi, &p.tmHin32, &hbar[ew], grp * 32, tw, b);
          tma_load_3d(piece_lo, &p.tmHin32, &hbar[ew], grp * 32, tw, p.B + b);
        }
#pragma unroll
        for (int ci = 0; ci < 2; ++ci) {
          const int cc = grp * 32 + ci * 16;
          uint32_t racc[16];
          tmem_ld16(taddr_rs + 128 + ci * 16, racc);
          tmem_ld_wait();
          if (last_block) {
            uint32_t hi2[8], lo2[8];
#pragma unroll
            for (int j = 0; j < 16; j += 2) {
              const float2 s0 = sb2[128 + cc + j], s1 = sb2[128 + cc + j + 1];
              const float y0 = old[ci * 16 + j] + fmaf(__uint_as_float(racc[j]), s0.x, s0.y);
              const float y1 = old[ci * 16 + j + 1] + fmaf(__uint_as_float(racc[j + 1]), s1.x, s1.y);
              split16x2(valid ? fmaxf(y0, 0.f) : 0.f, valid ? fmaxf(y1, 0.f) : 0.f, hi2[j >> 1], lo2[j >> 1]);
            }
            if (in_range) {
              __half* srow = p.skip16 + ((size_t)b * p.T + t) * 128 + cc;
#pragma unroll
              for (int v = 0; v < 2; ++v) {
                reinterpret_cast<uint4*>(srow)[v] = make_uint4(hi2[4 * v], hi2[4 * v + 1], hi2[4 * v + 2], hi2[4 * v + 3]);
                reinterpret_cast<uint4*>(srow + plane)[v] = make_uint4(lo2[4 * v], lo2[4 * v + 1], lo2[4 * v + 2], lo2[4 * v + 3]);
              }
            }
          } else if (in_range) {
#pragma unroll
            for (int j = 0; j < 16; ++j) {
              const float2 s2 = sb2[128 + cc + j];
              const float y = valid ? fmaf(__uint_as_float(racc[j]), s2.x, s2.y) : 0.f;
              float* dst = sp0 + (size_t)(ci * 16 + j) * p.T;
              if (p.skip_set) __stcs(dst, y);
              else asm volatile("red.global.add.f32 [%0], %1;" ::"l"(dst), "f"(y) : "memory");
            }
          }
        }
        mbar_wait(&hbar[ew], titer & 1);
#pragma unroll
        for (int ci = 0; ci < 2; ++ci) {
          const int cc = grp * 32 + ci * 16;
          uint32_t racc[16];
          tmem_ld16(taddr_rs + ci * 16, racc);
          const uint32_t off0 = lane * 64 + (((ci * 2) ^ ((lane >> 1) & 3)) << 4);
          const uint32_t off1 = lane * 64 + (((ci * 2 + 1) ^ ((lane >> 1) & 3)) << 4);
          uint4 hv[2], lv[2];
          hv[0] = *reinterpret_cast<const uint4*>(piece_hi + off0);
          hv[1] = *reinterpret_cast<const uint4*>(piece_hi + off1);
          lv[0] = *reinterpret_cast<const uint4*>(piece_lo + off0);
          lv[1] = *reinterpret_cast<const uint4*>(piece_lo + off1);
          tmem_ld_wait();
          if (ci == 1) {
            tc_fence_before();
            __syncwarp();
            if (lane == 0) pair_arrive(&acc_free[r0], crank);
          }
          const uint32_t* hp = reinterpret_cast<const uint32_t*>(hv);
          const uint32_t* lp = reinterpret_cast<const uint32_t*>(lv);
          uint32_t hi2[8], lo2[8];
#pragma unroll
          for (int j = 0; j < 16; j += 2) {
            const float2 s0 = sb2[cc + j], s1 = sb2[cc + j + 1];
            const float2 oh = unpack_h2(hp[j >> 1]), ol = unpack_h2(lp[j >> 1]);
            const float v0 = fmaf(__uint_as_float(racc[j]), s0.x, s0.y), v1 = fmaf(__uint_as_float(racc[j + 1]), s1.x, s1.y);
            const float n0 = valid ? ((oh.x + ol.x) + v0) * p.scale : 0.f;
            const float n1 = valid ? ((oh.y + ol.y) + v1) * p.scale : 0.f;
            split16x2(n0, n1, hi2[j >> 1], lo2[j >> 1]);
          }
          if constexpr (Q8) {
            if (in_range) {
              uint32_t qh[8], ql[8];
#pragma unroll
              for (int j = 0; j < 8; ++j) q8_pair(hi2[j], lo2[j], qh[j], ql[j]);
              uint8_t* d8 = p.h8_out + ((size_t)b * p.T + t) * 128 + cc;
              *reinterpret_cast<uint4*>(d8) = make_uint4(qh[0] | (qh[1] << 16), qh[2] | (qh[3] << 16), qh[4] | (qh[5] << 16), qh[6] | (qh[7] << 16));
              *reinterpret_cast<uint4*>(d8 + plane) = make_uint4(ql[0] | (ql[1] << 16), ql[2] | (ql[3] << 16), ql[4] | (ql[5] << 16), ql[6] | (ql[7] << 16));
            }
          }
          *reinterpret_cast<uint4*>(piece_hi + off0) = make_uint4(hi2[0], hi2[1], hi2[2], hi2[3]);
          *reinterpret_cast<uint4*>(piece_hi + off1) = make_uint4(hi2[4], hi2[5], hi2[6], hi2[7]);
          *reinterpret_cast<uint4*>(piece_lo + off0) = make_uint4(lo2[0], lo2[1], lo2[2], lo2[3]);
          *reinterpret_cast<uint4*>(piece_lo + off1) = make_uint4(lo2[4], lo2[5], lo2[6], lo2[7]);
        }
        fence_proxy_async();
        __syncwarp();
        if (lane == 0) {
          tma_store_3d(&p.tmHout32, piece_hi, grp * 32, tw, b);
          tma_store_3d(&p.tmHout32, piece_lo, grp * 32, tw, p.B + b);
          asm volatile("cp.async.bulk.commit_group;" ::: "memory");
        }
        if (STATS) st_acc[6] += clock64() - r_t0;
      }
    }
    asm volatile("cp.async.bulk.wait_group.read 0;" ::: "memory");
    if (STATS && p.stats && blockIdx.x == 0 && lane == 0 && (warp == 2 || warp == 10)) {
      unsigned long long* o = p.stats + (warp == 2 ? 11 : 19);
      for (int i = 0; i < 8; ++i) atomicAdd(o + i, (unsigned long long)st_acc[i]);
    }
  }
  tc_fence_before();
  __syncthreads();
  if constexpr (PAIR) cluster_sync_all();
  if (warp == 1) {
    tc_fence_after();
    if constexpr (PAIR) tmem_dealloc2(tmem_base, 512); else tmem_dealloc(tmem_base, 512);
  }
}

}
}
```

### tts_cube_b200/csrc/tc_conv.cuh

```cuda
#pragma once
#include <cuda_fp8.h>
#include <cuda.h>
#include <cuda_fp16.h>
#include <cuda_runtime.h>
#include <stdint.h>

namespace cube {
namespace tc {

constexpr int BM = 128;
constexpr int BN = 256;
#ifndef CUBE_TC_BK
#define CUBE_TC_BK 32
#endif
constexpr int BK = CUBE_TC_BK;
constexpr int STAGES = (BK == 64) ? 2 : 4;
constexpr int ROW_BYTES = BK * 2;
constexpr int SBO_BYTES = 8 * ROW_BYTES;
static_assert(BK == 64 || BK == 32, "BK must be 64 (SW128) or 32 (SW64)");
constexpr int A_TILE_BYTES = BM * BK * 2;
constexpr int B_TILE_BYTES = BN * BK * 2;
constexpr int STAGE_BYTES = 2 * A_TILE_BYTES + 2 * B_TILE_BYTES;

__host__ __device__ constexpr int swz_off(int r, int k) {
// ... 72 lines not shown
};

__device__ __forceinline__ uint32_t smem_u32(const void* p) { return (uint32_t)__cvta_generic_to_shared(p); }

__device__ __forceinline__ void mbar_init(uint64_t* bar, uint32_t count) {
  asm volatile("mbarrier.init.shared::cta.b64 [%0], %1;" ::"r"(smem_u32(bar)), "r"(count));
}
__device__ __forceinline__ void mbar_expect_tx(uint64_t* bar, uint32_t bytes) {
  asm volatile("mbarrier.arrive.expect_tx.shared::cta.b64 _, [%0], %1;" ::"r"(smem_u32(bar)), "r"(bytes) : "memory");
}
__device__ __forceinline__ void mbar_arrive(uint64_t* bar) {
  asm volatile("mbarrier.arrive.shared::cta.b64 _, [%0];" ::"r"(smem_u32(bar)) : "memory");
}
__device__ __forceinline__ uint32_t mbar_try_wait(uint64_t* bar, uint32_t parity) {
  uint32_t ok;
  asm volatile(
      "{\n\t"
      ".reg .pred p;\n\t"
      "mbarrier.try_wait.parity.shared::cta.b64 p, [%1], %2;\n\t"
      "selp.u32 %0, 1, 0, p;\n\t"
      "}"
      : "=r"(ok)
      : "r"(smem_u32(bar)), "r"(parity)
      : "memory");
  return ok;
}
__device__ __forceinline__ uint32_t mbar_test_wait(uint64_t* bar, uint32_t parity) {
  uint32_t ok;
  asm volatile(
      "{\n\t"
      ".reg .pred p;\n\t"
      "mbarrier.test_wait.parity.shared::cta.b64 p, [%1], %2;\n\t"
      "selp.u32 %0, 1, 0, p;\n\t"
      "}"
      : "=r"(ok)
      : "r"(smem_u32(bar)), "r"(parity)
      : "memory");
  return ok;
}
__device__ __forceinline__ void mbar_wait(uint64_t* bar, uint32_t parity) {
  while (!mbar_try_wait(bar, parity)) {
  }
}
__device__ __forceinline__ void fence_barrier_init() { asm volatile("fence.mbarrier_init.release.cluster;" ::: "memory"); }
__device__ __forceinline__ void fence_proxy_async() { asm volatile("fence.proxy.async.shared::cta;" ::: "memory"); }

__device__ __forceinline__ void tma_load_3d(void* dst, const CUtensorMap* tm, uint64_t* bar, int c0, int c1, int c2) {
  asm volatile(
      "cp.async.bulk.tensor.3d.shared::cluster.global.mbarrier::complete_tx::bytes [%0], [%1, {%3, %4, %5}], [%2];" ::"r"(smem_u32(dst)),
      "l"(reinterpret_cast<uint64_t>(tm)), "r"(smem_u32(bar)), "r"(c0), "r"(c1), "r"(c2)
      : "memory");
}
__device__ __forceinline__ void tma_store_3d(const CUtensorMap* tm, const void* src, int c0, int c1, int c2) {
  asm volatile("cp.async.bulk.tensor.3d.global.shared::cta.bulk_group [%0, {%2, %3, %4}], [%1];" ::"l"(reinterpret_cast<uint64_t>(tm)),
               "r"(smem_u32(src)), "r"(c0), "r"(c1), "r"(c2)
               : "memory");
}
__device__ __forceinline__ void bulk_load(void* dst, const void* src, uint32_t bytes, uint64_t* bar) {
  asm volatile("cp.async.bulk.shared::cluster.global.mbarrier::complete_tx::bytes [%0], [%1], %2, [%3];" ::"r"(smem_u32(dst)),
               "l"(reinterpret_cast<uint64_t>(src)), "r"(bytes), "r"(smem_u32(bar))
               : "memory");
}
__device__ __forceinline__ uint32_t mapa_u32(uint32_t addr, uint32_t rank) {
  uint32_t r;
  asm volatile("mapa.shared::cluster.u32 %0, %1, %2;" : "=r"(r) : "r"(addr), "r"(rank));
  return r;
}
__device__ __forceinline__ void tma_load_3d_bar(void* dst, const CUtensorMap* tm, uint32_t bar_addr, int c0, int c1, int c2) {
  asm volatile(
      "cp.async.bulk.tensor.3d.shared::cluster.global.mbarrier::complete_tx::bytes [%0], [%1, {%3, %4, %5}], [%2];" ::"r"(smem_u32(dst)),
      "l"(reinterpret_cast<uint64_t>(tm)), "r"(bar_addr), "r"(c0), "r"(c1), "r"(c2)
      : "memory");
}
__device__ __forceinline__ void bulk_load_bar(void* dst, const void* src, uint32_t bytes, uint32_t bar_addr) {
  asm volatile("cp.async.bulk.shared::cluster.global.mbarrier::complete_tx::bytes [%0], [%1], %2, [%3];" ::"r"(smem_u32(dst)),
               "l"(reinterpret_cast<uint64_t>(src)), "r"(bytes), "r"(bar_addr)
               : "memory");
}
__device__ __forceinline__ void prefetch_l2(const void* p) { asm volatile("prefetch.global.L2 [%0];" ::"l"(p)); }
__device__ __forceinline__ void prefetch_tmap(const CUtensorMap* tm) {
  asm volatile("prefetch.tensormap [%0];" ::"l"(reinterpret_cast<uint64_t>(tm)) : "memory");
}

__device__ __forceinline__ void tmem_alloc(uint32_t* dst_smem, uint32_t ncols) {
  asm volatile("tcgen05.alloc.cta_group::1.sync.aligned.shared::cta.b32 [%0], %1;" ::"r"(smem_u32(dst_smem)), "r"(ncols) : "memory");
  asm volatile("tcgen05.relinquish_alloc_permit.cta_group::1.sync.aligned;" ::: "memory");
}
__device__ __forceinline__ void tmem_dealloc(uint32_t taddr, uint32_t ncols) {
  asm volatile("tcgen05.dealloc.cta_group::1.sync.aligned.b32 %0, %1;" ::"r"(taddr), "r"(ncols) : "memory");
}
__device__ __forceinline__ void tc_fence_before() { asm volatile("tcgen05.fence::before_thread_sync;" ::: "memory"); }
__device__ __forceinline__ void tc_fence_after() { asm volatile("tcgen05.fence::after_thread_sync;" ::: "memory"); }

__device__ __forceinline__ void umma_f16(uint32_t tmem_d, uint64_t da, uint64_t db, uint32_t idesc, uint32_t accumulate) {
  asm volatile(
      "{\n\t"
      ".reg .pred p;\n\t"
      "setp.ne.b32 p, %4, 0;\n\t"
      "tcgen05.mma.cta_group::1.kind::f16 [%0], %1, %2, %3, p;\n\t"
      "}" ::"r"(tmem_d),
      "l"(da), "l"(db), "r"(idesc), "r"(accumulate)
      : "memory");
}
__device__ __forceinline__ void umma_commit(uint64_t* bar) {
  asm volatile("tcgen05.commit.cta_group::1.mbarrier::arrive::one.shared::cluster.b64 [%0];" ::"r"(smem_u32(bar)) : "memory");
}

__device__ __forceinline__ bool elect_one() {
  uint32_t pred;
  asm volatile(
      "{\n\t"
      ".reg .pred P;\n\t"
      "elect.sync _|P, 0xffffffff;\n\t"
      "selp.u32 %0, 1, 0, P;\n\t"
      "}"
      : "=r"(pred));
  return pred != 0;
}

__device__ __forceinline__ uint32_t cluster_ctarank() {
  uint32_t r;
  asm volatile("mov.u32 %0, %%cluster_ctarank;" : "=r"(r));
  return r;
}
__device__ __forceinline__ void cluster_sync_all() {
  asm volatile("barrier.cluster.arrive.release.aligned;" ::: "memory");
  asm volatile("barrier.cluster.wait.acquire.aligned;" ::: "memory");
}
__device__ __forceinline__ void mbar_arrive_remote(uint64_t* bar, uint32_t rank) {
  asm volatile(
      "{\n\t"
      ".reg .b32 ra;\n\t"
      "mapa.shared::cluster.u32 ra, %0, %1;\n\t"
      "mbarrier.arrive.relaxed.cluster.shared::cluster.b64 _, [ra];\n\t"
      "}" ::"r"(smem_u32(bar)), "r"(rank) : "memory");
}
__device__ __forceinline__ void tmem_alloc2(uint32_t* dst_smem, uint32_t ncols) {
  asm volatile("tcgen05.alloc.cta_group::2.sync.aligned.shared::cta.b32 [%0], %1;" ::"r"(smem_u32(dst_smem)), "r"(ncols) : "memory");
  asm volatile("tcgen05.relinquish_alloc_permit.cta_group::2.sync.aligned;" ::: "memory");
}
__device__ __forceinline__ void tmem_dealloc2(uint32_t taddr, uint32_t ncols) {
  asm volatile("tcgen05.dealloc.cta_group::2.sync.aligned.b32 %0, %1;" ::"r"(taddr), "r"(ncols) : "memory");
}
__device__ __forceinline__ void umma_f16_2(uint32_t tmem_d, uint64_t da, uint64_t db, uint32_t idesc, uint32_t accumulate) {
  asm volatile(
      "{\n\t"
      ".reg .pred p;\n\t"
      "setp.ne.b32 p, %4, 0;\n\t"
      "tcgen05.mma.cta_group::2.kind::f16 [%0], %1, %2, %3, p;\n\t"
      "}" ::"r"(tmem_d),
      "l"(da), "l"(db), "r"(idesc), "r"(accumulate)
      : "memory");
}
__device__ __forceinline__ void umma_commit_2(uint64_t* bar) {
  asm volatile("tcgen05.commit.cta_group::2.mbarrier::arrive::one.shared::cluster.multicast::cluster.b64 [%0], %1;" ::"r"(smem_u32(bar)),
               "h"((uint16_t)3)
               : "memory");
}

__device__ __forceinline__ void tmem_ld32(uint32_t taddr, uint32_t (&r)[32]) {
  asm volatile(
      "tcgen05.ld.sync.aligned.32x32b.x32.b32 "
      "{%0, %1, %2, %3, %4, %5, %6, %7, %8, %9, %10, %11, %12, %13, %14, %15, "
      "%16, %17, %18, %19, %20, %21, %22, %23, %24, %25, %26, %27, %28, %29, %30, %31}, [%32];"
      : "=r"(r[0]), "=r"(r[1]), "=r"(r[2]), "=r"(r[3]), "=r"(r[4]), "=r"(r[5]), "=r"(r[6]), "=r"(r[7]), "=r"(r[8]), "=r"(r[9]),
        "=r"(r[10]), "=r"(r[11]), "=r"(r[12]), "=r"(r[13]), "=r"(r[14]), "=r"(r[15]), "=r"(r[16]), "=r"(r[17]), "=r"(r[18]),
        "=r"(r[19]), "=r"(r[20]), "=r"(r[21]), "=r"(r[22]), "=r"(r[23]), "=r"(r[24]), "=r"(r[25]), "=r"(r[26]), "=r"(r[27]),
        "=r"(r[28]), "=r"(r[29]), "=r"(r[30]), "=r"(r[31])
      : "r"(taddr));
}
__device__ __forceinline__ void tmem_ld_wait() { asm volatile("tcgen05.wait::ld.sync.aligned;" ::: "memory"); }

__device__ __forceinline__ uint64_t make_desc(uint32_t smem_addr) {
  uint64_t d = 0;
  d |= (uint64_t)((smem_addr >> 4) & 0x3FFF);
  d |= (uint64_t)1 << 16;
  d |= (uint64_t)(SBO_BYTES >> 4) << 32;
  d |= (uint64_t)1 << 46;
  d |= (uint64_t)(BK == 64 ? 2 : 4) << 61;
  return d;
}

__device__ __forceinline__ uint64_t desc_add(uint64_t d, uint32_t byte_off) {
  return (d & 0xFFFFFFFF00000000ull) | (uint64_t)((uint32_t)d + (byte_off >> 4));
}

__host__ __device__ constexpr uint32_t make_idesc(int n, int m = BM) {
  return (1u << 4) | (0u << 7) | (0u << 10) | (0u << 15) | (0u << 16) | ((uint32_t)(n >> 3) << 17) | ((uint32_t)(m >> 4) << 24);
}

__host__ __device__ constexpr int swz32_off(int r, int k) { return r * 32 + ((((k >> 4) & 1) ^ ((r >> 2) & 1)) << 4) + (k & 15); }
__device__ __forceinline__ uint64_t make_desc32(uint32_t smem_addr) {
  uint64_t d = 0;
  d |= (uint64_t)((smem_addr >> 4) & 0x3FFF);
  d |= (uint64_t)1 << 16;
  d |= (uint64_t)((8 * 32) >> 4) << 32;
  d |= (uint64_t)1 << 46;
  d |= (uint64_t)6 << 61;
  return d;
}
__host__ __device__ constexpr uint32_t make_idesc_f8(int n, int m, int a_e5m2) {
  return (1u << 4) | ((uint32_t)a_e5m2 << 7) | (0u << 10) | ((uint32_t)(n >> 3) << 17) | ((uint32_t)(m >> 4) << 24);
}
__device__ __forceinline__ void umma_f8(uint32_t tmem_d, uint64_t da, uint64_t db, uint32_t idesc, uint32_t accumulate) {
  asm volatile(
      "{\n\t"
      ".reg .pred p;\n\t"
      "setp.ne.b32 p, %4, 0;\n\t"
      "tcgen05.mma.cta_group::1.kind::f8f6f4 [%0], %1, %2, %3, p;\n\t"
      "}" ::"r"(tmem_d),
      "l"(da), "l"(db), "r"(idesc), "r"(accumulate)
      : "memory");
}
__device__ __forceinline__ void q8_pair(uint32_t hi2, uint32_t lo2, uint32_t& q_hi, uint32_t& q_lo) {
  const float2 h = __half22float2(*reinterpret_cast<const __half2*>(&hi2));
  const float2 l = __half22float2(*reinterpret_cast<const __half2*>(&lo2));
  q_hi = __nv_cvt_float2_to_fp8x2(h, __NV_SATFINITE, __NV_E4M3);
  q_lo = __nv_cvt_float2_to_fp8x2(make_float2(l.x * 16.f, l.y * 16.f), __NV_SATFINITE, __NV_E5M2);
}

__device__ __forceinline__ __half f2h_sat(float x) {
  unsigned short r;
  asm("cvt.rn.satfinite.f16.f32 %0, %1;" : "=h"(r) : "f"(x));
  return __ushort_as_half(r);
}
__device__ __forceinline__ void split16(float x, __half& hi, __half& lo) {
  hi = f2h_sat(x);
  lo = f2h_sat(x - __half2float(hi));
}
__device__ __forceinline__ void tmem_ld16(uint32_t taddr, uint32_t (&r)[16]) {
  asm volatile(
      "tcgen05.ld.sync.aligned.32x32b.x16.b32 "
      "{%0, %1, %2, %3, %4, %5, %6, %7, %8, %9, %10, %11, %12, %13, %14, %15}, [%16];"
      : "=r"(r[0]), "=r"(r[1]), "=r"(r[2]), "=r"(r[3]), "=r"(r[4]), "=r"(r[5]), "=r"(r[6]), "=r"(r[7]), "=r"(r[8]), "=r"(r[9]),
        "=r"(r[10]), "=r"(r[11]), "=r"(r[12]), "=r"(r[13]), "=r"(r[14]), "=r"(r[15])
      : "r"(taddr));
}
__device__ __forceinline__ void tmem_ld8(uint32_t taddr, uint32_t (&r)[8]) {
  asm volatile("tcgen05.ld.sync.aligned.32x32b.x8.b32 {%0, %1, %2, %3, %4, %5, %6, %7}, [%8];"
               : "=r"(r[0]), "=r"(r[1]), "=r"(r[2]), "=r"(r[3]), "=r"(r[4]), "=r"(r[5]), "=r"(r[6]), "=r"(r[7])
               : "r"(taddr));
}
__device__ __forceinline__ float ex2_fast(float x) {
  float y;
  asm("ex2.approx.ftz.f32 %0, %1;" : "=f"(y) : "f"(x));
  return y;
}
__device__ __forceinline__ float rcp_fast(float x) {
  float y;
  asm("rcp.approx.ftz.f32 %0, %1;" : "=f"(y) : "f"(x));
  return y;
}
__device__ __forceinline__ uint32_t pack_h2_sat(float x0, float x1) {
  uint32_t r;
  asm("cvt.rn.satfinite.f16x2.f32 %0, %1, %2;" : "=r"(r) : "f"(x1), "f"(x0));
  return r;
}
__device__ __forceinline__ void split16x2(float x0, float x1, uint32_t& hi2, uint32_t& lo2) {
  hi2 = pack_h2_sat(x0, x1);
  const float2 hf = __half22float2(*reinterpret_cast<const __half2*>(&hi2));
  lo2 = pack_h2_sat(x0 - hf.x, x1 - hf.y);
}
__device__ __forceinline__ float2 unpack_h2(uint32_t v) { return __half22float2(*reinterpret_cast<const __half2*>(&v)); }

__device__ __forceinline__ float sigmoid_fast(float x) { return __fdividef(1.f, 1.f + __expf(-x)); }
__device__ __forceinline__ float tanh_fast(float x) { return 1.f - __fdividef(2.f, 1.f + __expf(2.f * x)); }

template <int TN, bool CG2 = false, bool WIN = false, int MS = 0>
__global__ void __launch_bounds__(NUM_THREADS, 1) tc_conv_kernel(const __grid_constant__ TcParams p) {
  static_assert(!(CG2 && WIN), "window mode is single-CTA");
  static_assert(!(CG2 && MS > 0), "the sub-tile override is single-CTA");
  constexpr int SA = WinCfg<TN, MS>::SA, SB = WinCfg<TN, MS>::SB;
  constexpr int A_SLOT = WinCfg<TN, MS>::A_SLOT, B_SLOT = WinCfg<TN, MS>::B_SLOT;
  constexpr int A_LO_OFF = WinCfg<TN, MS>::NBOX * A_TILE_BYTES;
  constexpr int STAGES = WIN ? (SA + SB + 1) / 2 : Cfg<TN, CG2, MS>::NSTAGE;
  constexpr int STAGE_BYTES = WIN ? (SA * A_SLOT + SB * B_SLOT + STAGES - 1) / STAGES : Cfg<TN, CG2, MS>::STAGE;
  constexpr int B_TILE_BYTES = Cfg<TN, CG2, MS>::B_BYTES;
  constexpr int BN = TN;
  constexpr bool CAT = Cfg<TN, CG2, MS>::CAT;
  constexpr int ACCW = Cfg<TN, CG2, MS>::ACC_COLS;
  constexpr int MSUB = Cfg<TN, CG2, MS>::MSUB;
  constexpr int A_BYTES = Cfg<TN, CG2, MS>::A_BYTES;
  constexpr int CTA_ROWS = MSUB * BM;
  constexpr int TILE_ROWS = CG2 ? 2 * CTA_ROWS : CTA_ROWS;
  extern __shared__ uint8_t smem_raw[];
  uint8_t* smem = reinterpret_cast<uint8_t*>((reinterpret_cast<uintptr_t>(smem_raw) + 1023) & ~(uintptr_t)1023);
  constexpr int DATA_BYTES = WIN ? SA * A_SLOT + SB * B_SLOT : STAGES * STAGE_BYTES;
  uint64_t* bars = reinterpret_cast<uint64_t*>(smem + DATA_BYTES);
  uint64_t* full = bars;
  uint64_t* empty = bars + STAGES;
  uint64_t* pfull = bars + 2 * STAGES;
  uint64_t* fullA = bars, *emptyA = bars + SA, *fullB = bars + 2 * SA, *emptyB = bars + 2 * SA + SB;
  constexpr int NB_RING = WIN ? 2 * SA + 2 * SB : 3 * STAGES;
  uint64_t* tfull = bars + NB_RING;
  uint64_t* tempty = bars + NB_RING + 2;
  uint32_t* tmem_slot = reinterpret_cast<uint32_t*>(bars + NB_RING + 4);
  static_assert((NB_RING + 4) * 8 + 4 <= 256, "barrier block");
  const uint32_t crank = CG2 ? cluster_ctarank() : 0u;
  const int tile0 = CG2 ? (int)(blockIdx.x >> 1) : (int)blockIdx.x;
  const int tile_step = CG2 ? (int)(gridDim.x >> 1) : (int)gridDim.x;
  float2* s_sb = reinterpret_cast<float2*>(smem + DATA_BYTES + 256);

  const int warp = threadIdx.x >> 5, lane = threadIdx.x & 31;
  const int nphase = p.nphase > 0 ? p.nphase : 1;
  const int total_tiles = p.n_tiles * p.t_tiles * p.B * nphase;

  if (warp == 0 && lane == 0) {
    prefetch_tmap(&p.tmA[0]);
    if (p.nseg > 1) prefetch_tmap(&p.tmA[1]);
// ... 97 lines not shown
      auto kstep = [&](uint32_t d_tmem, uint32_t ao, uint32_t bo, int ks, uint32_t acc) {
        const uint32_t ko = ks * 32;
#pragma unroll
        for (int ms = 0; ms < MSUB; ++ms) {
          const uint32_t a = ao + ms * A_TILE_BYTES + ko;
          const uint32_t d = d_tmem + ms * ACCW;
          if constexpr (CAT) {
            umma_f16(d, desc_add(D16, a), desc_add(D16, bo + ko), idesc_cat, acc);
            umma_f16(d, desc_add(D16, a + A_LO_OFF), desc_add(D16, bo + ko), idesc, 1);
          } else {
            umma_f16(d, desc_add(D16, a), desc_add(D16, bo + ko), idesc, acc);
            umma_f16(d, desc_add(D16, a), desc_add(D16, bo + B_SLOT / 2 + ko), idesc, 1);
            umma_f16(d, desc_add(D16, a + A_LO_OFF), desc_add(D16, bo + ko), idesc, 1);
          }
        }
      };
      for (int tile = tile0; tile < total_tiles; tile += tile_step, ++titer) {
        const uint32_t acc = titer & 1, aph = (titer >> 1) & 1;
        mbar_wait(&tempty[acc], aph ^ 1);
        tc_fence_after();
        const uint32_t d_tmem = tmem_u + acc * (MSUB * ACCW);
        uint32_t accumulate = 0;
        for (int s = 0; s < p.nseg; ++s) {
          const int taps = p.seg[s].taps, nchunks = p.seg[s].nchunks, last_ksteps = p.seg[s].last_ksteps;
          const uint32_t tap_bytes = (uint32_t)p.seg[s].dil * ROW_BYTES;
          for (int cc = 0; cc < nchunks; ++cc) {
            mbar_wait(&fullA[sa], pha);
            const int ksteps = cc != nchunks - 1 ? BK / 16 : last_ksteps;
            uint32_t ao = sa * A_SLOT;
            for (int tap = 0; tap < taps; ++tap, ao += tap_bytes) {
              mbar_wait(&fullB[sbi], phb);
              tc_fence_after();
              const uint32_t bo = SA * A_SLOT + sbi * B_SLOT;
              if (leader) {
#pragma unroll
                for (int ks = 0; ks < BK / 16; ++ks)
                  if (ks < ksteps) kstep(d_tmem, ao, bo, ks, ks ? 1u : accumulate);
                umma_commit(&emptyB[sbi]);
              }
              accumulate = 1;
              if (++sbi == SB) { sbi = 0; phb ^= 1; }
            }
            if (leader) umma_commit(&emptyA[sa]);
            if (++sa == SA) { sa = 0; pha ^= 1; }
          }
        }
        if (leader) umma_commit(&tfull[acc]);
      }
    } else if (lane == 0) {
      if (CG2 && crank != 0) {
        uint32_t it = 0;
        for (int tile = tile0; tile < total_tiles; tile += tile_step) {
          for (int s = 0; s < p.nseg; ++s) {
            const TcSeg sg = p.seg[s];
            for (int n = sg.taps * sg.nchunks; n > 0; --n, ++it) {
              const int st = it % STAGES;
              mbar_wait(&full[st], (it / STAGES) & 1);
              mbar_arrive_remote(&pfull[st], 0);
            }
          }
        }
      } else if (WIN) {
        constexpr uint32_t idesc = make_idesc(TN, BM);
        constexpr uint32_t idesc_cat = make_idesc(CAT ? 2 * TN : TN, BM);
        uint32_t ia = 0, ib = 0, titer = 0;
        for (int tile = tile0; tile < total_tiles; tile += tile_step, ++titer) {
          const uint32_t acc = titer & 1, aph = (titer >> 1) & 1;
          mbar_wait(&tempty[acc], aph ^ 1);
          tc_fence_after();
          const uint32_t d_tmem = tmem_base + acc * (MSUB * ACCW);
          uint32_t accumulate = 0;
          for (int s = 0; s < p.nseg; ++s) {
            const TcSeg sg = p.seg[s];
            for (int cc = 0; cc < sg.nchunks; ++cc, ++ia) {
              const int sa = ia % SA;
              mbar_wait(&fullA[sa], (ia / SA) & 1);
              const uint32_t a_base = smem_u32(smem + sa * A_SLOT);
              const int ksteps = (cc == sg.nchunks - 1) ? sg.last_ksteps : (BK / 16);
              for (int tap = 0; tap < sg.taps; ++tap, ++ib) {
                const int sbi = ib % SB;
                mbar_wait(&fullB[sbi], (ib / SB) & 1);
                tc_fence_after();
                const uint32_t b_hi = smem_u32(smem + SA * A_SLOT + sbi * B_SLOT);
                const uint32_t a_tap = a_base + (uint32_t)(tap * sg.dil) * ROW_BYTES;
                const uint64_t dah = make_desc(a_tap), dal = make_desc(a_tap + A_LO_OFF), dbh = make_desc(b_hi), dbl = make_desc(b_hi + B_SLOT / 2);
                for (int ks = 0; ks < ksteps; ++ks) {
                  const uint32_t ko = ks * 32;
#pragma unroll
                  for (int ms = 0; ms < MSUB; ++ms) {
                    const uint32_t ao = ms * A_TILE_BYTES + ko;
                    const uint32_t d = d_tmem + ms * ACCW;
                    if constexpr (CAT) {
                      umma_f16(d, desc_add(dah, ao), desc_add(dbh, ko), idesc_cat, accumulate);
                      umma_f16(d, desc_add(dal, ao), desc_add(dbh, ko), idesc, 1);
                    } else {
                      umma_f16(d, desc_add(dah, ao), desc_add(dbh, ko), idesc, accumulate);
                      umma_f16(d, desc_add(dah, ao), desc_add(dbl, ko), idesc, 1);
                      umma_f16(d, desc_add(dal, ao), desc_add(dbh, ko), idesc, 1);
                    }
                  }
                  accumulate = 1;
                }
                umma_commit(&emptyB[sbi]);
              }
              umma_commit(&emptyA[sa]);
            }
          }
          umma_commit(&tfull[acc]);
        }
      } else {
        constexpr uint32_t idesc = make_idesc(TN, CG2 ? 2 * BM : BM);
        constexpr uint32_t idesc_cat = make_idesc(CAT ? 2 * TN : TN, BM);
        uint32_t it = 0, titer = 0;
        for (int tile = tile0; tile < total_tiles; tile += tile_step, ++titer) {
          const uint32_t acc = titer & 1, aph = (titer >> 1) & 1;
          mbar_wait(&tempty[acc], aph ^ 1);
          tc_fence_after();
          const uint32_t d_tmem = tmem_base + acc * (MSUB * ACCW);
          uint32_t accumulate = 0;
          for (int s = 0; s < p.nseg; ++s) {
            const TcSeg sg = p.seg[s];
            for (int tap = 0; tap < sg.taps; ++tap) {
              for (int cc = 0; cc < sg.nchunks; ++cc, ++it) {
                const int st = it % STAGES;
                const uint32_t par = (it / STAGES) & 1;
                mbar_wait(&full[st], par);
                if constexpr (CG2) mbar_wait(&pfull[st], par);
                tc_fence_after();
                const uint32_t a_hi0 = smem_u32(smem + st * STAGE_BYTES);
                const uint32_t b_hi = a_hi0 + 2 * A_BYTES;
                const uint32_t b_lo = b_hi + B_TILE_BYTES;
                const int ksteps = (cc == sg.nchunks - 1) ? sg.last_ksteps : (BK / 16);
                for (int ks = 0; ks < ksteps; ++ks) {
                  const uint32_t ko = ks * 32;
#pragma unroll
                  for (int ms = 0; ms < MSUB; ++ms) {
                    const uint32_t a_hi = a_hi0 + ms * A_TILE_BYTES, a_lo = a_hi + A_BYTES;
                    const uint32_t d = d_tmem + ms * ACCW;
                    if constexpr (CAT) {
                      umma_f16(d, make_desc(a_hi + ko), make_desc(b_hi + ko), idesc_cat, accumulate);
                      umma_f16(d, make_desc(a_lo + ko), make_desc(b_hi + ko), idesc, 1);
                    } else if constexpr (CG2) {
                      umma_f16_2(d, make_desc(a_hi + ko), make_desc(b_hi + ko), idesc, accumulate);
                      umma_f16_2(d, make_desc(a_hi + ko), make_desc(b_lo + ko), idesc, 1);
                      umma_f16_2(d, make_desc(a_lo + ko), make_desc(b_hi + ko), idesc, 1);
                    } else {
                      umma_f16(d, make_desc(a_hi + ko), make_desc(b_hi + ko), idesc, accumulate);
                      umma_f16(d, make_desc(a_hi + ko), make_desc(b_lo + ko), idesc, 1);
                      umma_f16(d, make_desc(a_lo + ko), make_desc(b_hi + ko), idesc, 1);
                    }
                  }
                  accumulate = 1;
                }
                if constexpr (CG2) umma_commit_2(&empty[st]); else umma_commit(&empty[st]);
              }
            }
          }
          if constexpr (CG2) umma_commit_2(&tfull[acc]); else umma_commit(&tfull[acc]);
        }
      }
    }
  } else {
    constexpr float LOG2E = 1.4426950408889634f;
    const int q = warp & 3;
    const int grp = (warp - 2) >> 2;
    const int msub = grp % MSUB;
    const int sub = grp / MSUB;
    const int row = q * 32 + lane;
    const int etid = threadIdx.x - 64;
    uint32_t titer = 0;
    int sb_nt = -1;
    for (int tile = tile0; tile < total_tiles; tile += tile_step, ++titer) {
      const int nt = tile % p.n_tiles;
      int rest = tile / p.n_tiles;
      const int ph = rest % nphase; rest /= nphase;
      const int tt = rest % p.t_tiles, b = rest / p.t_tiles;
      const int t = p.row0 + tt * TILE_ROWS + (int)crank * CTA_ROWS + msub * BM + row;
      const uint32_t acc = titer & 1, aph = (titer >> 1) & 1;
      if (nt != sb_nt) {
        asm volatile("bar.sync 1, 512;" ::: "memory");
        if (etid < BN) {
          float sc = __ldg(p.inv_scale + nt * BN + etid) * p.a_inv_scale, bi = __ldg(p.bias + nt * BN + etid);
          if (p.epi == TC_EPI_GATE) {
            const float k = etid < BN / 2 ? 2.f * LOG2E : -LOG2E;
            sc *= k; bi *= k;
          }
          s_sb[etid] = make_float2(sc, bi);
        }
        asm volatile("bar.sync 1, 512;" ::: "memory");
        sb_nt = nt;
      }
      const uint32_t taddr = tmem_base + (acc * MSUB + msub) * ACCW + ((uint32_t)(q * 32) << 16);
      const int len = p.lens ? min(p.lens[b], p.T) : p.T;
      const bool in_range = t < p.T;
      const bool valid = t < len;
      if (in_range) {
        if (p.epi == TC_EPI_CONV) {
          if (p.res16) {
            const int t_out = t * p.ostride + p.ooff[ph];
            if (t_out >= 0 && t_out < p.L_out) {
              const __half* r0 = p.res16 + ((size_t)b * p.L_out + t_out) * p.outC + nt * BN + sub * (BN * MSUB / 4);
              prefetch_l2(r0);
              prefetch_l2(r0 + (size_t)p.B * p.L_out * p.outC);
            }
          }
        } else if (p.epi == TC_EPI_RESSKIP) {
          if (sub < 2) {
            const __half* h0 = p.h16 + ((size_t)b * p.T + t) * p.hC + sub * 64;
            prefetch_l2(h0);
            prefetch_l2(h0 + (size_t)p.B * p.T * p.hC);
          } else if (!p.skip_set && (lane & 7) == 0) {
            const float* s0 = p.skip + ((size_t)b * (BN / 2) + (sub - 2) * 64) * p.T + t;
#pragma unroll 8
            for (int j = 0; j < 64; ++j) prefetch_l2(s0 + (size_t)j * p.T);
          }
        }
      }
      mbar_wait(&tfull[acc], aph);
      tc_fence_after();
      if (p.epi == TC_EPI_CONV) {
        constexpr int CPS = BN * MSUB / 4;
        constexpr int CW = CPS < 16 ? CPS : 16;
        const int t_out = t * p.ostride + p.ooff[ph];
        const int olen = p.lens ? min(p.lens[b], p.L_out) : p.L_out;
        const bool o_in = in_range && t_out >= 0 && t_out < p.L_out;
        const bool o_valid = o_in && t_out < olen;
        const size_t rowoff = ((size_t)b * p.L_out + (o_in ? t_out : 0)) * p.outC + nt * BN;
        const size_t plane = (size_t)p.B * p.L_out * p.outC;
#pragma unroll
        for (int cc = sub * CPS; cc < sub * CPS + CPS; cc += CW) {
          uint32_t r[CW];
          if constexpr (CW == 16) tmem_ld16(taddr + cc, r); else tmem_ld8(taddr + cc, r);
          uint32_t r2[CAT ? CW : 1];
          if constexpr (CAT) { if constexpr (CW == 16) tmem_ld16(taddr + BN + cc, r2); else tmem_ld8(taddr + BN + cc, r2); }
          uint32_t rh[CW / 2], rl[CW / 2];
          float old[CW];
          if (p.res16 && o_in) {
#pragma unroll
            for (int v = 0; v < CW / 8; ++v) {
              const uint4 a = reinterpret_cast<const uint4*>(p.res16 + rowoff + cc)[v];
              const uint4 c = reinterpret_cast<const uint4*>(p.res16 + plane + rowoff + cc)[v];
              rh[4 * v] = a.x; rh[4 * v + 1] = a.y; rh[4 * v + 2] = a.z; rh[4 * v + 3] = a.w;
              rl[4 * v] = c.x; rl[4 * v + 1] = c.y; rl[4 * v + 2] = c.z; rl[4 * v + 3] = c.w;
            }
          } else {
#pragma unroll
            for (int v = 0; v < CW / 2; ++v) rh[v] = rl[v] = 0u;
          }
          if (p.acc32 && p.acc_mode >= TC_ACC_ADD && o_in) {
#pragma unroll
            for (int j = 0; j < CW; ++j) old[j] = __ldcs(p.acc32 + ((size_t)b * p.outC + nt * BN + cc + j) * p.L_out + t_out);
          } else {
#pragma unroll
            for (int j = 0; j < CW; ++j) old[j] = 0.f;
          }
          tmem_ld_wait();
          if constexpr (CAT) {
#pragma unroll
            for (int j = 0; j < CW; ++j) r[j] = __float_as_uint(__uint_as_float(r[j]) + __uint_as_float(r2[j]));
          }
          float v[CW];
#pragma unroll
          for (int j = 0; j < CW; j += 2) {
            const float2 s0 = s_sb[cc + j], s1 = s_sb[cc + j + 1];
            const float2 ah = unpack_h2(rh[j >> 1]), al = unpack_h2(rl[j >> 1]);
            float a0 = (ah.x + al.x) * p.a_inv_scale, a1 = (ah.y + al.y) * p.a_inv_scale;
            a0 = a0 < 0.f ? a0 * p.res_inv_slope : a0;
            a1 = a1 < 0.f ? a1 * p.res_inv_slope : a1;
            v[j] = o_valid ? fmaf(__uint_as_float(r[j]), s0.x, s0.y) + a0 : 0.f;
            v[j + 1] = o_valid ? fmaf(__uint_as_float(r[j + 1]), s1.x, s1.y) + a1 : 0.f;
          }
          if (p.out16 && o_in) {
            uint32_t hi2[CW / 2], lo2[CW / 2];
#pragma unroll
            for (int j = 0; j < CW; j += 2) {
              const float y0 = v[j] < 0.f ? v[j] * p.out_slope : v[j], y1 = v[j + 1] < 0.f ? v[j + 1] * p.out_slope : v[j + 1];
              split16x2(y0 * p.plane_scale, y1 * p.plane_scale, hi2[j >> 1], lo2[j >> 1]);
            }
#pragma unroll
            for (int q4 = 0; q4 < CW / 8; ++q4) {
              reinterpret_cast<uint4*>(p.out16 + rowoff + cc)[q4] = make_uint4(hi2[4 * q4], hi2[4 * q4 + 1], hi2[4 * q4 + 2], hi2[4 * q4 + 3]);
              reinterpret_cast<uint4*>(p.out16 + plane + rowoff + cc)[q4] = make_uint4(lo2[4 * q4], lo2[4 * q4 + 1], lo2[4 * q4 + 2], lo2[4 * q4 + 3]);
            }
          }
          if (p.acc32 && o_in) {
            if (p.acc_mode == TC_ACC_ADD_DIV) {
#pragma unroll
              for (int j = 0; j < CW; ++j) v[j] = o_valid ? (old[j] + v[j]) / p.acc_div : 0.f;
              if (p.acc_store) {
#pragma unroll
                for (int j = 0; j < CW; ++j) __stcs(p.acc32 + ((size_t)b * p.outC + nt * BN + cc + j) * p.L_out + t_out, v[j]);
              }
              if (p.out16b) {
                uint32_t hi2[CW / 2], lo2[CW / 2];
#pragma unroll
                for (int j = 0; j < CW; j += 2) {
                  const float y0 = v[j] < 0.f ? v[j] * p.out_slope : v[j], y1 = v[j + 1] < 0.f ? v[j + 1] * p.out_slope : v[j + 1];
                  split16x2(y0 * p.plane_scale, y1 * p.plane_scale, hi2[j >> 1], lo2[j >> 1]);
                }
#pragma unroll
                for (int q4 = 0; q4 < CW / 8; ++q4) {
                  reinterpret_cast<uint4*>(p.out16b + rowoff + cc)[q4] = make_uint4(hi2[4 * q4], hi2[4 * q4 + 1], hi2[4 * q4 + 2], hi2[4 * q4 + 3]);
                  reinterpret_cast<uint4*>(p.out16b + plane + rowoff + cc)[q4] = make_uint4(lo2[4 * q4], lo2[4 * q4 + 1], lo2[4 * q4 + 2], lo2[4 * q4 + 3]);
                }
              }
            } else {
#pragma unroll
              for (int j = 0; j < CW; ++j) __stcs(p.acc32 + ((size_t)b * p.outC + nt * BN + cc + j) * p.L_out + t_out, old[j] + v[j]);
            }
          }
        }
// ... 216 lines not shown
```

### tts_cube_b200/generator.py

```python
from __future__ import annotations

import ctypes as C
from typing import Dict, List, Mapping, Optional, Sequence, Tuple

import torch

from . import _lib
from ._lib import VocConfig, check, lib
from .streaming import HifiganStream, step_streams


def _cfg_get(h, key, default=None):
    if isinstance(h, Mapping):
        return h.get(key, default)
    return getattr(h, key, default)


def _stream_ptr(device: torch.device) -> int:
    return torch.cuda.current_stream(device).cuda_stream


class _Handle:

    def __init__(self, cfg: VocConfig, device: torch.device):
        self.ptr = C.c_void_p()
        self.device = device
        self.num_mels = int(cfg.num_mels)
        check(lib().cube_voc_create(C.byref(self.ptr), C.byref(cfg), device.index or 0))

    def load(self, sd: Mapping[str, torch.Tensor]) -> None:
        for name, t in sd.items():
            a = t.detach().to("cpu", torch.float32).contiguous()
            shape = (C.c_int64 * max(a.dim(), 1))(*a.shape)
            check(lib().cube_voc_load_weight(self.ptr, name.encode(), C.c_void_p(a.data_ptr()), shape, a.dim()))

    def finalize(self) -> None:
        check(lib().cube_voc_finalize(self.ptr))

    def out_len(self, n_frames: int) -> int:
        n = lib().cube_voc_out_len(self.ptr, int(n_frames))
        if n < 0:
            check(1)
        return int(n)

    def forward(self, mel: torch.Tensor, n_frames: Optional[Sequence[int]], noise: Optional[torch.Tensor],
                want_int16: bool = False):
        if mel.device.type != "cuda":
            raise _lib.CubeVocError("mel must live on a CUDA device (no CPU path)")
        if mel.dtype != torch.float32 or mel.dim() != 3:
            raise _lib.CubeVocError(f"mel must be float32 [B, C, F], got {mel.dtype} {tuple(mel.shape)}")
        self._check_shapes(mel, n_frames)
        if mel.device != self.device:
            raise _lib.CubeVocError(f"mel lives on {mel.device} but this vocoder's weights live on {self.device}")
        mel = mel.contiguous()
        B, _, F = mel.shape
        T = self.out_len(F)
        wav = torch.empty(B, 1, T, device=mel.device, dtype=torch.float32)
        w16 = torch.empty(B, T, device=mel.device, dtype=torch.int16) if want_int16 else None
        nf = None
        if n_frames is not None:
            nf = (C.c_int32 * B)(*[int(v) for v in n_frames])
        if noise is not None:
            noise = noise.to(mel.device, torch.float32).contiguous()
            if noise.numel() != B * T:
                raise _lib.CubeVocError(f"noise must have B*T={B * T} elements, got {noise.numel()}")
        with torch.cuda.device(mel.device):
            check(lib().cube_voc_forward(
                self.ptr, C.c_void_p(mel.data_ptr()), nf, C.c_void_p(noise.data_ptr()) if noise is not None else None,
                C.c_void_p(wav.data_ptr()), C.c_void_p(w16.data_ptr()) if w16 is not None else None,
                B, F, C.c_void_p(_stream_ptr(mel.device))))
        return (wav, w16) if want_int16 else wav

    def forward_range(self, mel: torch.Tensor, n_frames: Optional[Sequence[int]], begin: Sequence[int],
                      end: Sequence[int], want_int16: bool = False, out: Optional[torch.Tensor] = None):
        if mel.device.type != "cuda" or mel.dtype != torch.float32 or mel.dim() != 3:
            raise _lib.CubeVocError(f"mel must be float32 [B, C, F] on a CUDA device, got {mel.dtype} {tuple(mel.shape)} on {mel.device}")
        self._check_shapes(mel, n_frames)
        if mel.device != self.device:
            raise _lib.CubeVocError(f"mel lives on {mel.device} but this vocoder's weights live on {self.device}")
        mel = mel.contiguous()
        B, _, F = mel.shape
        if len(begin) != B or len(end) != B:
            raise _lib.CubeVocError(f"begin / end need {B} entries, got {len(begin)} / {len(end)}")
        T = self.out_len(F)
        shape, dt = ((B, T), torch.int16) if want_int16 else ((B, 1, T), torch.float32)
        if out is None:
            out = torch.empty(*shape, device=mel.device, dtype=dt)
        elif tuple(out.shape) != shape or out.dtype != dt or out.device != mel.device or not out.is_contiguous():
            raise _lib.CubeVocError(f"`out` must be a contiguous {dt} {shape} tensor on {mel.device}")
        nf = (C.c_int32 * B)(*[int(v) for v in n_frames]) if n_frames is not None else None
        b0 = (C.c_int64 * B)(*[int(v) for v in begin])
        b1 = (C.c_int64 * B)(*[int(v) for v in end])
        wav = None
        if want_int16:
            wav = torch.empty(B, 1, T, device=mel.device, dtype=torch.float32)
        with torch.cuda.device(mel.device):
            check(lib().cube_voc_forward_range(
                self.ptr, C.c_void_p(mel.data_ptr()), nf, b0, b1,
                C.c_void_p((wav if want_int16 else out).data_ptr()), C.c_void_p(out.data_ptr()) if want_int16 else None,
                B, F, C.c_void_p(_stream_ptr(mel.device))))
        flat = out.view(B, T)
        return out, [flat[b, int(begin[b]):int(end[b])] for b in range(B)]

    def _check_shapes(self, mel: torch.Tensor, n_frames) -> None:
        if mel.shape[1] != self.num_mels:
            raise _lib.CubeVocError(f"mel has {mel.shape[1]} channels, this vocoder was built for num_mels={self.num_mels}")
        if mel.shape[0] < 1 or mel.shape[2] < 1:
            raise _lib.CubeVocError(f"empty batch {tuple(mel.shape)}")
        if n_frames is not None and len(n_frames) != mel.shape[0]:
            raise _lib.CubeVocError(f"n_frames has {len(n_frames)} entries for a batch of {mel.shape[0]}")

    def forward_host(self, mel: torch.Tensor, n_frames, noise: Optional[torch.Tensor], out: torch.Tensor):
        if mel.dim() != 3:
            raise _lib.CubeVocError(f"mel must be [B, C, F], got {tuple(mel.shape)}")
        for name, t in (("mel", mel), ("noise", noise), ("out", out)):
            if t is None:
                continue
            if t.device.type != "cpu" or not t.is_contiguous():
                raise _lib.CubeVocError(f"forward_host takes contiguous HOST tensors; `{name}` is {t.device}, contiguous={t.is_contiguous()}")
        if mel.dtype != torch.float32 or (noise is not None and noise.dtype != torch.float32):
            raise _lib.CubeVocError("forward_host takes float32 mel / noise")
        if out.dtype not in (torch.float32, torch.int16):
            raise _lib.CubeVocError(f"`out` must be float32 or int16, got {out.dtype}")
        self._check_shapes(mel, n_frames)
        B, _, F = mel.shape
        T = self.out_len(F)
        if out.numel() != B * T:
            raise _lib.CubeVocError(f"`out` must hold B*T = {B}*{T} samples, got {tuple(out.shape)}")
        if noise is not None and noise.numel() != B * T:
            raise _lib.CubeVocError(f"noise must have B*T = {B * T} elements, got {noise.numel()}")
        nf = (C.c_int32 * B)(*[int(v) for v in n_frames]) if n_frames is not None else None
        wav_p = C.c_void_p(out.data_ptr()) if out.dtype == torch.float32 else None
        i16_p = C.c_void_p(out.data_ptr()) if out.dtype == torch.int16 else None
        check(lib().cube_voc_forward_host(self.ptr, C.c_void_p(mel.data_ptr()), nf,
                                          C.c_void_p(noise.data_ptr()) if noise is not None else None,
                                          wav_p, i16_p, B, F))
        return out

    def launches(self) -> int:
        return int(lib().cube_voc_last_launches(self.ptr))

    def workspace_bytes(self) -> int:
        return int(lib().cube_voc_workspace_bytes(self.ptr))

    def set_profile(self, on: bool) -> None:
        check(lib().cube_voc_set_profile(self.ptr, int(on)))

    def get_profile(self) -> Dict[str, float]:
        cap = 64
        names = C.create_string_buffer(cap * 64)
        ms = (C.c_float * cap)()
        n = lib().cube_voc_get_profile(self.ptr, names, ms, cap)
        if n < 0:
            check(1)
        return {names.raw[i * 64:(i + 1) * 64].split(b"\0")[0].decode(): float(ms[i]) for i in range(n)}

    def close(self):
        if self.ptr:
            lib().cube_voc_destroy(self.ptr)
            self.ptr = C.c_void_p()

    def __del__(self):
        try:
            self.close()
        except Exception:
            pass


def hifigan_tc_supported(h) -> bool:
    c0 = int(_cfg_get(h, "upsample_initial_channel"))
    n = len(list(_cfg_get(h, "upsample_rates")))
    widths = [c0 >> i for i in range(n + 1)]
    return (str(_cfg_get(h, "resblock")) == "1" and all(w in (32, 64, 128, 256, 512) for w in widths)
            and int(_cfg_get(h, "num_mels", 80) or 80) % 8 == 0)


def hifigan_config(h, math=None) -> VocConfig:
    if math is None:
        math = _lib.MATH_TC_SPLIT16 if hifigan_tc_supported(h) else _lib.MATH_FP32_SIMT
    cfg = VocConfig()
    cfg.arch = _lib.ARCH_HIFIGAN
    cfg.math = math
    cfg.num_mels = int(_cfg_get(h, "num_mels", 80) or 80)
    cfg.upsample_initial_channel = int(_cfg_get(h, "upsample_initial_channel"))
    rates = list(_cfg_get(h, "upsample_rates"))
    ks = list(_cfg_get(h, "upsample_kernel_sizes"))
    if len(rates) != len(ks) or len(rates) > _lib.MAX_UPS:
        raise _lib.CubeVocError("bad upsample_rates / upsample_kernel_sizes")
    cfg.n_ups = len(rates)
    for i, (u, k) in enumerate(zip(rates, ks)):
        cfg.upsample_rates[i], cfg.upsample_kernel_sizes[i] = int(u), int(k)
    cfg.resblock_type = 1 if str(_cfg_get(h, "resblock")) == "1" else 2
    rk = list(_cfg_get(h, "resblock_kernel_sizes"))
    rd = list(_cfg_get(h, "resblock_dilation_sizes"))
    cfg.n_resblock_kernels = len(rk)
    for j, (k, d) in enumerate(zip(rk, rd)):
        cfg.resblock_kernel_sizes[j] = int(k)
        cfg.n_dilations[j] = len(d)
        for m, dd in enumerate(d):
            cfg.resblock_dilations[j][m] = int(dd)
    return cfg


class CubeGenerator(torch.nn.Module):

    def __init__(self, h, math=None):
        super().__init__()
        self.h = h
        self._cfg = hifigan_config(h, math)
        self._sd: Dict[str, torch.Tensor] = {}
        self._handle: Optional[_Handle] = None
        self.register_buffer("_device_tracker", torch.zeros(1), persistent=False)
        lib()

    def load_state_dict(self, state_dict, strict: bool = True, assign: bool = False):
        sd = {k: v for k, v in state_dict.items()}
        self._sd = {k: v.detach().to("cpu", torch.float32).clone() for k, v in sd.items()}
        self._drop_handle()
        return torch.nn.modules.module._IncompatibleKeys([], [])

    def state_dict(self, *a, **k):
        return dict(self._sd)

    def remove_weight_norm(self):
        return self

    def _drop_handle(self):
        if self._handle is not None:
            self._handle.close()
            self._handle = None

    def _apply(self, fn, *a, **k):
        before = self._device_tracker.device
        r = super()._apply(fn, *a, **k)
        if self._device_tracker.device != before:
            self._drop_handle()
        return r

    @property
    def device(self) -> torch.device:
        return self._device_tracker.device

    def _ensure(self) -> _Handle:
        if self._handle is None:
            dev = self.device
            if dev.type != "cuda":
                raise _lib.CubeVocError("CubeGenerator must be moved to a CUDA device (.to('cuda:0')); there is no CPU path")
            if not self._sd:
                raise _lib.CubeVocError("load_state_dict() must be called before forward()")
            dev = torch.device("cuda", dev.index if dev.index is not None else torch.cuda.current_device())
            hd = _Handle(self._cfg, dev)
            hd.load(self._sd)
            hd.finalize()
            self._handle = hd
        return self._handle

    def out_len(self, n_frames: int) -> int:
        return self._ensure().out_len(n_frames)

    def forward(self, x: torch.Tensor, n_frames: Optional[Sequence[int]] = None) -> torch.Tensor:
        if torch.is_grad_enabled() and x.requires_grad:
            raise _lib.CubeVocError("CubeGenerator is inference-only: call it under torch.no_grad() "
                                    "(training goes through the reference Generator)")
        return self._ensure().forward(x, n_frames, None)

    def forward_int16(self, x: torch.Tensor, n_frames: Optional[Sequence[int]] = None):
        return self._ensure().forward(x, n_frames, None, want_int16=True)

    @property
    def hop(self) -> int:
        n = 1
        for i in range(self._cfg.n_ups):
            n *= int(self._cfg.upsample_rates[i])
        return n

    def sample_support(self, s0: int, s1: int) -> Tuple[int, int]:
        f0, f1 = C.c_int64(), C.c_int64()
        check(lib().cube_voc_hifigan_support(C.byref(self._cfg), int(s0), int(s1), C.byref(f0), C.byref(f1)))
        return int(f0.value), int(f1.value)

    def forward_range(self, mel: torch.Tensor, n_frames: Optional[Sequence[int]], begin: Sequence[int],
                      end: Sequence[int], int16: bool = False, out: Optional[torch.Tensor] = None) -> List[torch.Tensor]:
        return self._ensure().forward_range(mel, n_frames, begin, end, want_int16=int16, out=out)[1]

    def open_stream(self, int16: bool = False) -> HifiganStream:
        return HifiganStream(self.sample_support, self.out_len, self.hop, int(self._cfg.num_mels), int16=int16, owner=self)

    def step_streams(self, streams: Sequence[HifiganStream]) -> List[torch.Tensor]:
        out: List[Optional[torch.Tensor]] = [None] * len(streams)
        for i16 in (False, True):
            idx = [i for i, s in enumerate(streams) if s.int16 == i16]
            if not idx:
                continue
            vr = lambda m, nf, b, e, i16=i16: self.forward_range(m, nf, b, e, int16=i16)
            for i, piece in zip(idx, step_streams([streams[i] for i in idx], vr, device=self.device)):
                out[i] = piece
        return out
# ... 20 lines not shown
```

Baseline: 14.70 million.

## Multicast block weights across clusters of 2 or 4 CTA pairs

Extends the CTA-pair block kernel so a cluster can hold 1, 2 or 4 pairs. Each pair loads only a slice of the shared weight tile and multicasts it to the matching CTAs in the other pairs, cutting duplicate global/L2 weight traffic. The empty barriers now wait on all pairs and the t-tile count is padded to a multiple of the cluster width. A host heuristic picks the width from occupancy-derived cluster counts, which adds cross-pair coupling, extra drain waits and possible padding waste.

```diff
diff --git a/include/cube_vocoder.h b/include/cube_vocoder.h
--- a/include/cube_vocoder.h
+++ b/include/cube_vocoder.h
@@ -84,6 +84,8 @@
 
 int64_t cube_voc_last_launches(const cube_voc_t* h);
 int64_t cube_voc_workspace_bytes(const cube_voc_t* h);
+int cube_voc_set_block_mcast(cube_voc_t* h, int pairs_per_cluster);
+int cube_voc_last_block_mcast(const cube_voc_t* h);
 int cube_voc_set_profile(cube_voc_t* h, int on);
 int cube_voc_get_profile(cube_voc_t* h, char* names , float* ms, int cap);
 
diff --git a/tts_cube_b200/_lib.py b/tts_cube_b200/_lib.py
--- a/tts_cube_b200/_lib.py
+++ b/tts_cube_b200/_lib.py
@@ -71,6 +71,8 @@
     "cube_wavernn_max_batch": (C.c_int, [_P]),
     "cube_voc_last_launches": (C.c_int64, [_P]),
     "cube_voc_workspace_bytes": (C.c_int64, [_P]),
+    "cube_voc_set_block_mcast": (C.c_int, [_P, C.c_int]),
+    "cube_voc_last_block_mcast": (C.c_int, [_P]),
     "cube_voc_set_profile": (C.c_int, [_P, C.c_int]),
     "cube_voc_get_profile": (C.c_int, [_P, _P, _P, C.c_int]),
     "cube_voc_destroy": (None, [_P]),
diff --git a/tts_cube_b200/csrc/engine.cu b/tts_cube_b200/csrc/engine.cu
--- a/tts_cube_b200/csrc/engine.cu
+++ b/tts_cube_b200/csrc/engine.cu
@@ -6,6 +6,7 @@
 
 #include <map>
 #include <string>
+#include <type_traits>
 #include <vector>
 
 #include "../../include/cube_vocoder.h"
@@ -97,6 +98,8 @@
   int* h_lens_pin = nullptr; size_t h_lens_pin_cap = 0;
   bool lens_from_pinned = false;
   int sm_count = 148;
+  int block_mcast = 0;
+  int block_mcast_req = 0;
   bool profile = false;
   std::vector<ProfRec> prof;
   PackedConv conv_pre, conv_post_w;
@@ -1014,6 +1017,51 @@
   static int v = -1;
   if (v < 0) { const char* e = getenv("CUBE_TC_LEAN"); v = e ? (e[0] == '1' ? 1 : 0) : CUBE_LEAN_DEFAULT; }
   return v == 1;
+}
+
+template <int MC>
+static int block_clusters(int device) {
+  static std::map<int, int> cache;
+  auto it = cache.find(device);
+  if (it != cache.end()) return it->second;
+  auto kernel = tc::tc_block_kernel<true, true, false, false, MC>;
+  int n = 0;
+  cudaLaunchConfig_t cfg;
+  memset(&cfg, 0, sizeof(cfg));
+  cudaLaunchAttribute at[1];
+  at[0].id = cudaLaunchAttributeClusterDimension;
+  at[0].val.clusterDim.x = 2 * MC; at[0].val.clusterDim.y = 1; at[0].val.clusterDim.z = 1;
+  cfg.attrs = at; cfg.numAttrs = 1;
+  cfg.gridDim = dim3(2 * MC); cfg.blockDim = dim3(tc::NUM_THREADS); cfg.dynamicSmemBytes = tc::PAIR_SMEM;
+  if (cudaFuncSetAttribute(kernel, cudaFuncAttributeMaxDynamicSharedMemorySize, tc::PAIR_SMEM) != cudaSuccess ||
+      cudaOccupancyMaxActiveClusters(&n, kernel, &cfg) != cudaSuccess) {
+    cudaGetLastError();
+    n = 0;
+  }
+  cache[device] = n;
+  return n;
+}
+
+static const double kMcastPeriod[3] = {1.0, 1.0, 1.0};
+
+static int block_mcast_pick(int device, int forced, int t_tiles, int B, int* clusters) {
+  const int n[3] = {block_clusters<1>(device), block_clusters<2>(device), block_clusters<4>(device)};
+  const int widths[3] = {1, 2, 4};
+  int best = 0;
+  if (forced) {
+    best = forced == 4 ? 2 : forced - 1;
+    while (best > 0 && n[best] <= 0) --best;
+  } else {
+    double best_cost = 0;
+    for (int k = 0; k < 3; ++k) {
+      if (n[k] <= 0) continue;
+      const long long groups = (long long)((t_tiles + widths[k] - 1) / widths[k]) * B;
+      const double cost = (double)((groups + n[k] - 1) / n[k]) * kMcastPeriod[k];
+      if (k == 0 || cost < best_cost) { best = k; best_cost = cost; }
+    }
+  }
+  *clusters = n[best];
+  return widths[best];
 }
 
 static bool use_cg2() {
@@ -1506,6 +1554,13 @@
         static int aonce = -1;
         if (aonce < 0) { const char* e = getenv("CUBE_TC_AONCE"); aonce = (e && e[0] == '1') ? 1 : 0; }
         const bool use_aonce = pairv == 1 && aonce == 1 && !stats;
+        int mc = 1, clusters = h->sm_count / 2;
+        if (pairv == 1) {
+          bp.t_tiles = (T + 2 * tc::BM - 1) / (2 * tc::BM);
+          if (!use_aonce) mc = block_mcast_pick(h->device, h->block_mcast_req, bp.t_tiles, B, &clusters);
+          bp.t_tiles = (bp.t_tiles + mc - 1) / mc * mc;
+        }
+        h->block_mcast = pairv == 1 ? mc : 0;
         auto launch = [&](auto kernel, bool pair) -> int {
           const size_t smem = use_aonce ? tc::AONCE_SMEM : (pair ? tc::PAIR_SMEM : tc::BLK_SMEM);
           static std::map<std::pair<const void*, int>, bool> attr_done;
@@ -1518,11 +1573,10 @@
           memset(&cfg, 0, sizeof(cfg));
           cudaLaunchAttribute at[1];
           if (pair) {
-            bp.t_tiles = (T + 2 * tc::BM - 1) / (2 * tc::BM);
-            const long long ptiles = (long long)bp.t_tiles * B;
-            cfg.gridDim = dim3(2 * (unsigned)std::min<long long>(ptiles, h->sm_count / 2));
+            const long long groups = (long long)bp.t_tiles / mc * B;
+            cfg.gridDim = dim3(2 * mc * (unsigned)std::min<long long>(groups, std::max(clusters, 1)));
             at[0].id = cudaLaunchAttributeClusterDimension;
-            at[0].val.clusterDim.x = 2; at[0].val.clusterDim.y = 1; at[0].val.clusterDim.z = 1;
+            at[0].val.clusterDim.x = 2 * mc; at[0].val.clusterDim.y = 1; at[0].val.clusterDim.z = 1;
             cfg.attrs = at; cfg.numAttrs = 1;
           } else {
             const long long tiles = (long long)bp.t_tiles * B;
@@ -1538,8 +1592,13 @@
         if (use_aonce) {
           lrc = q8 ? launch(tc::tc_block_kernel<true, true, false, true>, true) : launch(tc::tc_block_kernel<true, false, false, true>, true);
         } else if (pairv == 1) {
-          if (stats) lrc = q8 ? launch(tc::tc_block_kernel<true, true, true>, true) : launch(tc::tc_block_kernel<true, false, true>, true);
-          else lrc = q8 ? launch(tc::tc_block_kernel<true, true, false>, true) : launch(tc::tc_block_kernel<true, false, false>, true);
+          auto launch_mc = [&](auto mct) -> int {
+            constexpr int M = decltype(mct)::value;
+            if (stats) return q8 ? launch(tc::tc_block_kernel<true, true, true, false, M>, true) : launch(tc::tc_block_kernel<true, false, true, false, M>, true);
+            return q8 ? launch(tc::tc_block_kernel<true, true, false, false, M>, true) : launch(tc::tc_block_kernel<true, false, false, false, M>, true);
+          };
+          lrc = mc == 4 ? launch_mc(std::integral_constant<int, 4>()) : mc == 2 ? launch_mc(std::integral_constant<int, 2>())
+                                                                              : launch_mc(std::integral_constant<int, 1>());
         } else {
           if (stats) lrc = q8 ? launch(tc::tc_block_kernel<false, true, true>, false) : launch(tc::tc_block_kernel<false, false, true>, false);
           else lrc = q8 ? launch(tc::tc_block_kernel<false, true, false>, false) : launch(tc::tc_block_kernel<false, false, false>, false);
@@ -2177,6 +2236,17 @@
 
 int64_t cube_voc_last_launches(const cube_voc_t* h) { return h ? h->launches : -1; }
 
+int cube_voc_set_block_mcast(cube_voc_t* h, int pairs_per_cluster) {
+  if (!h) return fail("null handle");
+  if (pairs_per_cluster != 0 && pairs_per_cluster != 1 && pairs_per_cluster != 2 && pairs_per_cluster != 4)
+    return fail("pairs per cluster must be 0 (automatic), 1, 2 or 4, got %d", pairs_per_cluster);
+  h->block_mcast_req = pairs_per_cluster;
+  ++h->alloc_gen;
+  return 0;
+}
+
+int cube_voc_last_block_mcast(const cube_voc_t* h) { return h ? h->block_mcast : -1; }
+
 int64_t cube_voc_workspace_bytes(const cube_voc_t* h) {
   if (!h) return -1;
   int64_t n = 0;
diff --git a/tts_cube_b200/csrc/tc_block.cuh b/tts_cube_b200/csrc/tc_block.cuh
--- a/tts_cube_b200/csrc/tc_block.cuh
+++ b/tts_cube_b200/csrc/tc_block.cuh
@@ -66,8 +66,8 @@
       "l"(da), "l"(db), "r"(idesc), "r"(accumulate)
       : "memory");
 }
-__device__ __forceinline__ void pair_arrive(uint64_t* bar, uint32_t crank) {
-  if (crank == 0) mbar_arrive(bar); else mbar_arrive_remote(bar, 0);
+__device__ __forceinline__ void pair_arrive(uint64_t* bar, uint32_t half, uint32_t lead) {
+  if (half == 0) mbar_arrive(bar); else mbar_arrive_remote(bar, lead);
 }
 
 template <bool PAIR>
@@ -79,12 +79,27 @@
   if constexpr (PAIR) umma_f8_2(d, da, db, idesc, acc); else umma_f8(d, da, db, idesc, acc);
 }
 template <bool PAIR>
-__device__ __forceinline__ void blk_commit(uint64_t* bar) {
-  if constexpr (PAIR) umma_commit_2(bar); else umma_commit(bar);
-}
-
-template <bool PAIR, bool Q8, bool STATS = false, bool AONCE = false>
+__device__ __forceinline__ void blk_commit(uint64_t* bar, uint16_t cta_mask) {
+  if constexpr (PAIR) umma_commit_2(bar, cta_mask); else umma_commit(bar);
+}
+
+template <int MC, int WB>
+__device__ __forceinline__ void blk_weight_piece(uint8_t* wb, uint32_t off, const void* src, uint32_t bytes, uint32_t fbar, uint32_t j,
+                                                 uint16_t cta_mask) {
+  if constexpr (MC == 1) {
+    bulk_load_bar(wb + off, src, bytes, fbar);
+  } else {
+    constexpr uint32_t SL = WB / MC;
+    static_assert(WB % (MC * 16) == 0, "bulk copies move multiples of 16 bytes");
+    const uint32_t a = max(off, j * SL), e = min(off + bytes, j * SL + SL);
+    if (a < e) bulk_load_mc(wb + a, reinterpret_cast<const uint8_t*>(src) + (a - off), e - a, fbar, cta_mask);
+  }
+}
+
+template <bool PAIR, bool Q8, bool STATS = false, bool AONCE = false, int MC = 1>
 __global__ void __launch_bounds__(NUM_THREADS, 1) tc_block_kernel(const __grid_constant__ BlockParams p) {
+  static_assert(MC == 1 || MC == 2 || MC == 4, "1, 2 or 4 CTA pairs per cluster");
+  static_assert(MC == 1 || (PAIR && !AONCE), "weight multicast is a mode of the CTA-pair tiling");
   long long st_acc[STATS ? 8 : 1] = {0};
   const long long st_begin = STATS ? clock64() : 0;
   (void)st_acc; (void)st_begin;
@@ -97,7 +112,13 @@
   constexpr int TILE_ROWS = BlkCfg<PAIR>::TILE_ROWS;
   constexpr int NARR = PAIR ? 2 * NUM_EPI_WARPS : NUM_EPI_WARPS;
   const uint32_t crank = PAIR ? cluster_ctarank() : 0u;
-  const int tile0 = PAIR ? (int)(blockIdx.x >> 1) : (int)blockIdx.x;
+  const uint32_t half = MC > 1 ? crank & 1u : crank;
+  const uint32_t lead = MC > 1 ? crank & ~1u : 0u;
+  const uint16_t pmask = (uint16_t)(3u << lead);
+  constexpr uint16_t EMASK = (uint16_t)((1u << (2 * MC)) - 1);
+  constexpr uint16_t PARMASK = (uint16_t)(0x5555u & EMASK);
+  (void)PARMASK;
+  const int tile0 = !PAIR ? (int)blockIdx.x : (MC > 1 ? (int)((blockIdx.x / (2 * MC)) * MC + (crank >> 1)) : (int)(blockIdx.x >> 1));
   const int tile_step = PAIR ? (int)(gridDim.x >> 1) : (int)gridDim.x;
   extern __shared__ uint8_t smem_raw[];
   uint8_t* smem = reinterpret_cast<uint8_t*>((reinterpret_cast<uintptr_t>(smem_raw) + 1023) & ~(uintptr_t)1023);
@@ -122,7 +143,7 @@
   if (warp == 0 && lane == 0) {
     prefetch_tmap(&p.tmH);
     prefetch_tmap(&p.tmC);
-    for (int s = 0; s < NST; ++s) { mbar_init(&full[s], 1); mbar_init(&empty[s], 1); mbar_init(&pfull[s], 1); }
+    for (int s = 0; s < NST; ++s) { mbar_init(&full[s], 1); mbar_init(&empty[s], MC); mbar_init(&pfull[s], 1); }
     for (int r = 0; r < 2; ++r) { mbar_init(&acc_full[r], 1); mbar_init(&acc_free[r], NARR); }
     mbar_init(o_full, NARR);
     mbar_init(o_free, 1);
@@ -152,7 +173,7 @@
       uint32_t it = 0;
       for (int tile = tile0; tile < total_tiles; tile += tile_step) {
         const int tt = tile % p.t_tiles, b = tile / p.t_tiles;
-        const int t0 = tt * TILE_ROWS + (int)crank * BM;
+        const int t0 = tt * TILE_ROWS + (int)half * BM;
         for (int pass = 0; pass < NPASS; ++pass) {
           int chunk = 0;
           for (int tap = 0; tap <= p.taps; ++tap) {
@@ -180,13 +201,14 @@
                 uint8_t* wb = sb + 2 * A_TILE_BYTES + k * 2 * B_BYTES;
                 if constexpr (Q8) {
                   const uint8_t* wq = p.W1q + ((size_t)nt * nch1 + chunk) * 32768;
-                  bulk_load_bar(wb, wq + crank * B_BYTES, B_BYTES, fbar);
-                  bulk_load_bar(wb + B_BYTES, wq + 16384 + crank * (B_BYTES / 2), B_BYTES / 2, fbar);
-                  bulk_load_bar(wb + B_BYTES + B_BYTES / 2, wq + 24576 + crank * (B_BYTES / 2), B_BYTES / 2, fbar);
+                  blk_weight_piece<MC, 2 * B_BYTES>(wb, 0, wq + half * B_BYTES, B_BYTES, fbar, crank >> 1, PARMASK << half);
+                  blk_weight_piece<MC, 2 * B_BYTES>(wb, B_BYTES, wq + 16384 + half * (B_BYTES / 2), B_BYTES / 2, fbar, crank >> 1, PARMASK << half);
+                  blk_weight_piece<MC, 2 * B_BYTES>(wb, B_BYTES + B_BYTES / 2, wq + 24576 + half * (B_BYTES / 2), B_BYTES / 2, fbar, crank >> 1,
+                                                    PARMASK << half);
                 } else {
-                  const __half* wc = p.W1 + ((size_t)nt * nch1 + chunk) * 2 * (BN * BK) + (size_t)crank * (BN / 2) * BK ;
-                  bulk_load_bar(wb, wc, B_BYTES, fbar);
-                  bulk_load_bar(wb + B_BYTES, wc + BN * BK, B_BYTES, fbar);
+                  const __half* wc = p.W1 + ((size_t)nt * nch1 + chunk) * 2 * (BN * BK) + (size_t)half * (BN / 2) * BK ;
+                  blk_weight_piece<MC, 2 * B_BYTES>(wb, 0, wc, B_BYTES, fbar, crank >> 1, PARMASK << half);
+                  blk_weight_piece<MC, 2 * B_BYTES>(wb, B_BYTES, wc + BN * BK, B_BYTES, fbar, crank >> 1, PARMASK << half);
                 }
               }
             }
@@ -198,10 +220,13 @@
           uint8_t* sb = smem + st * STG;
           const uint32_t fbar = smem_u32(&full[st]);
           mbar_expect_tx(&full[st], 2 * B_BYTES);
-          const __half* wc = p.W2 + (size_t)ch * 2 * (BN * BK) + (size_t)crank * (BN / 2) * BK ;
-          bulk_load_bar(sb + 2 * A_TILE_BYTES, wc, B_BYTES, fbar);
-          bulk_load_bar(sb + 2 * A_TILE_BYTES + B_BYTES, wc + BN * BK, B_BYTES, fbar);
-        }
+          const __half* wc = p.W2 + (size_t)ch * 2 * (BN * BK) + (size_t)half * (BN / 2) * BK ;
+          blk_weight_piece<MC, 2 * B_BYTES>(sb + 2 * A_TILE_BYTES, 0, wc, B_BYTES, fbar, crank >> 1, PARMASK << half);
+          blk_weight_piece<MC, 2 * B_BYTES>(sb + 2 * A_TILE_BYTES, B_BYTES, wc + BN * BK, B_BYTES, fbar, crank >> 1, PARMASK << half);
+        }
+      }
+      if constexpr (MC > 1) {
+        for (int n = 0; n < NST; ++n, ++it) mbar_wait(&empty[it % NST], ((it / NST) & 1) ^ 1);
       }
       if (STATS && p.stats && blockIdx.x == 0) {
         atomicAdd(p.stats + 0, (unsigned long long)st_acc[0]);
@@ -210,7 +235,7 @@
       }
     }
   } else if (warp == 1) {
-    if (crank == 0 && p.lean) {
+    if (half == 0 && p.lean) {
       constexpr uint32_t idesc = make_idesc(BN, TILE_ROWS);
       constexpr uint32_t idesc8_0 = make_idesc_f8(BN, TILE_ROWS, 0), idesc8_1 = make_idesc_f8(BN, TILE_ROWS, 1);
       (void)idesc8_0; (void)idesc8_1;
@@ -264,14 +289,14 @@
                   }
                 }
               }
-              blk_commit<PAIR>(&empty[st]);
+              blk_commit<PAIR>(&empty[st], EMASK);
             }
             accumulate = 1;
             if (++st == NST) { st = 0; ph ^= 1; }
           }
           if (leader) {
 #pragma unroll
-            for (int k = 0; k < NTP; ++k) blk_commit<PAIR>(&acc_full[(AONCE ? k : pass) == 0 ? r0 : r1]);
+            for (int k = 0; k < NTP; ++k) blk_commit<PAIR>(&acc_full[(AONCE ? k : pass) == 0 ? r0 : r1], pmask);
           }
         }
         {
@@ -297,27 +322,27 @@
                   blk_mma_f16<PAIR>(d_tmem, desc_add(D16, ao + ko), desc_add(D16, bo + B_BYTES + ko), idesc, 1);
                   blk_mma_f16<PAIR>(d_tmem, desc_add(D16, ao + A8 + ko), desc_add(D16, bo + ko), idesc, 1);
                 }
-                blk_commit<PAIR>(&empty[st]);
+                blk_commit<PAIR>(&empty[st], EMASK);
               }
               accumulate = 1;
               if (++st == NST) { st = 0; ph ^= 1; }
             }
-            if (leader) blk_commit<PAIR>(o_free);
-          }
-          if (leader) blk_commit<PAIR>(&acc_full[r0]);
+            if (leader) blk_commit<PAIR>(o_free, pmask);
+          }
+          if (leader) blk_commit<PAIR>(&acc_full[r0], pmask);
         }
       }
       if (STATS && p.stats && blockIdx.x == 0 && leader) {
         for (int i = 0; i < 7; ++i) atomicAdd(p.stats + 3 + i, (unsigned long long)st_acc[i]);
         atomicAdd(p.stats + 10, (unsigned long long)(clock64() - st_begin));
       }
-    } else if (lane == 0 && crank != 0) {
+    } else if (lane == 0 && half != 0) {
       uint32_t it = 0;
       for (int tile = tile0; tile < total_tiles; tile += tile_step)
         for (int n = NPASS * nch1 + 8; n > 0; --n, ++it) {
           const int st = it % NST;
           mbar_wait(&full[st], (it / NST) & 1);
-          mbar_arrive_remote(&pfull[st], 0);
+          mbar_arrive_remote(&pfull[st], lead);
         }
     } else if (lane == 0) {
       constexpr uint32_t idesc = make_idesc(BN, TILE_ROWS);
@@ -371,11 +396,11 @@
                 }
               }
               accumulate = 1;
-              blk_commit<PAIR>(&empty[st]);
-            }
-          }
-#pragma unroll
-          for (int k = 0; k < NTP; ++k) blk_commit<PAIR>(&acc_full[(AONCE ? k : pass) == 0 ? r0 : r1]);
+              blk_commit<PAIR>(&empty[st], EMASK);
+            }
+          }
+#pragma unroll
+          for (int k = 0; k < NTP; ++k) blk_commit<PAIR>(&acc_full[(AONCE ? k : pass) == 0 ? r0 : r1], pmask);
         }
         {
           BLK_WAIT(&acc_free[r0], (free_ph[r0] & 1) ^ 1, 3);
@@ -400,11 +425,11 @@
                 blk_mma_f16<PAIR>(d_tmem, make_desc(a_lo + ko), make_desc(b_hi + ko), idesc, 1);
                 accumulate = 1;
               }
-              blk_commit<PAIR>(&empty[st]);
-            }
-            blk_commit<PAIR>(o_free);
-          }
-          blk_commit<PAIR>(&acc_full[r0]);
+              blk_commit<PAIR>(&empty[st], EMASK);
+            }
+            blk_commit<PAIR>(o_free, pmask);
+          }
+          blk_commit<PAIR>(&acc_full[r0], pmask);
         }
       }
       if (STATS && p.stats && blockIdx.x == 0) {
@@ -421,14 +446,14 @@
     uint32_t ofree_ph = 0;
     for (int tile = tile0; tile < total_tiles; tile += tile_step, ++titer) {
       const int tt = tile % p.t_tiles, b = tile / p.t_tiles;
-      const int t = tt * TILE_ROWS + (int)crank * BM + row;
+      const int t = tt * TILE_ROWS + (int)half * BM + row;
       const int r0 = titer & 1, r1 = r0 ^ 1;
       const int len = p.lens ? min(p.lens[b], p.T) : p.T;
       const bool in_range = t < p.T, valid = t < len;
       if (p.prefetch_next && tile + tile_step < total_tiles) {
         const int ntile = tile + tile_step;
         const int ntt = ntile % p.t_tiles, nb = ntile / p.t_tiles;
-        const int nt0 = ntt * TILE_ROWS + (int)crank * BM;
+        const int nt0 = ntt * TILE_ROWS + (int)half * BM;
         const int e = (int)threadIdx.x - 64;
         const int rr = e & 127, part = e >> 7;
         const size_t hplane = (size_t)p.B * p.T * 128;
@@ -494,7 +519,7 @@
         }
         tc_fence_before();
         __syncwarp();
-        if (lane == 0) pair_arrive(&acc_free[rg], crank);
+        if (lane == 0) pair_arrive(&acc_free[rg], half, lead);
         if (STATS) st_acc[5] += clock64() - g_t0;
         BLK_WAIT(o_free, (ofree_ph & 1) ^ 1, 2 + nt);
         ++ofree_ph;
@@ -514,7 +539,7 @@
         }
         fence_proxy_async();
         __syncwarp();
-        if (lane == 0) pair_arrive(o_full, crank);
+        if (lane == 0) pair_arrive(o_full, half, lead);
       }
       {
         const uint32_t taddr_rs = tmem_base + r0 * BN + ((uint32_t)(q * 32) << 16) + grp * 32;
@@ -524,7 +549,7 @@
         const int ew = warp - 2;
         uint8_t* piece_hi = o_smem + grp * 2 * A_TILE_BYTES + q * 2048;
         uint8_t* piece_lo = piece_hi + A_TILE_BYTES;
-        const int tw = tt * TILE_ROWS + (int)crank * BM + q * 32;
+        const int tw = tt * TILE_ROWS + (int)half * BM + q * 32;
         float old[32];
         if (last_block) {
 #pragma unroll
@@ -590,7 +615,7 @@
           if (ci == 1) {
             tc_fence_before();
             __syncwarp();
-            if (lane == 0) pair_arrive(&acc_free[r0], crank);
+            if (lane == 0) pair_arrive(&acc_free[r0], half, lead);
           }
           const uint32_t* hp = reinterpret_cast<const uint32_t*>(hv);
           const uint32_t* lp = reinterpret_cast<const uint32_t*>(lv);
diff --git a/tts_cube_b200/csrc/tc_conv.cuh b/tts_cube_b200/csrc/tc_conv.cuh
--- a/tts_cube_b200/csrc/tc_conv.cuh
+++ b/tts_cube_b200/csrc/tc_conv.cuh
@@ -248,9 +248,14 @@
       "l"(da), "l"(db), "r"(idesc), "r"(accumulate)
       : "memory");
 }
-__device__ __forceinline__ void umma_commit_2(uint64_t* bar) {
+__device__ __forceinline__ void umma_commit_2(uint64_t* bar, uint16_t cta_mask) {
   asm volatile("tcgen05.commit.cta_group::2.mbarrier::arrive::one.shared::cluster.multicast::cluster.b64 [%0], %1;" ::"r"(smem_u32(bar)),
-               "h"((uint16_t)3)
+               "h"(cta_mask)
+               : "memory");
+}
+__device__ __forceinline__ void bulk_load_mc(void* dst, const void* src, uint32_t bytes, uint32_t bar_addr, uint16_t cta_mask) {
+  asm volatile("cp.async.bulk.shared::cluster.global.mbarrier::complete_tx::bytes.multicast::cluster [%0], [%1], %2, [%3], %4;" ::"r"(smem_u32(dst)),
+               "l"(reinterpret_cast<uint64_t>(src)), "r"(bytes), "r"(bar_addr), "h"(cta_mask)
                : "memory");
 }
 
@@ -654,11 +659,11 @@
                   }
                   accumulate = 1;
                 }
-                if constexpr (CG2) umma_commit_2(&empty[st]); else umma_commit(&empty[st]);
+                if constexpr (CG2) umma_commit_2(&empty[st], 3); else umma_commit(&empty[st]);
               }
             }
           }
-          if constexpr (CG2) umma_commit_2(&tfull[acc]); else umma_commit(&tfull[acc]);
+          if constexpr (CG2) umma_commit_2(&tfull[acc], 3); else umma_commit(&tfull[acc]);
         }
       }
     }
diff --git a/tts_cube_b200/generator.py b/tts_cube_b200/generator.py
--- a/tts_cube_b200/generator.py
+++ b/tts_cube_b200/generator.py
@@ -143,6 +143,12 @@
     def workspace_bytes(self) -> int:
         return int(lib().cube_voc_workspace_bytes(self.ptr))
 
+    def set_block_mcast(self, pairs_per_cluster: int) -> None:
+        check(lib().cube_voc_set_block_mcast(self.ptr, int(pairs_per_cluster)))
+
+    def last_block_mcast(self) -> int:
+        return int(lib().cube_voc_last_block_mcast(self.ptr))
+
     def set_profile(self, on: bool) -> None:
         check(lib().cube_voc_set_profile(self.ptr, int(on)))
 
```

After: 14.68 million, median of 6. No clear change (-0.1%).
